# wg-perception/PartsBasedDetector

Measured on AMD Instinct MI355X. Metric: detect() frames/sec, 640x480, 26-part person model, higher is better.
Workload: dtype f32

## Files before the change

### partsbaseddetector_amd/csrc/fold_pick.hpp

```cpp
#pragma once
#include <math.h>

#ifdef __HIPCC__
#define FP_HD __host__ __device__ __forceinline__
#else
#define FP_HD static inline
#endif

template <typename T> struct FoldPick { T v; int i; };

template <typename T, int N = 0>
FP_HD FoldPick<T> fold_pick(const T* sd, const float* bias_col, int K) {
  const int n = N > 0 ? N : K;
  const T w0 = sd[0] + bias_col[0];
  T v = w0 > (T)-INFINITY ? w0 : (T)-INFINITY;
  int bi = 0;
#ifdef __HIPCC__
#pragma unroll
#endif
  for (int k = 1; k < n; ++k) {
    const T wv = sd[k] + bias_col[k];
    const bool take = wv > v;
    bi = take ? k : bi;
    v = take ? wv : v;
  }
  return FoldPick<T>{K == 1 ? w0 : v, bi};
}
```

### partsbaseddetector_amd/csrc/k_dp.hip

```cpp
#include <algorithm>
#include <type_traits>
#include "pbd_internal.hpp"
#include "dt_core.hpp"
#include "fold_pick.hpp"

#define GP(U) const __attribute__((address_space(1))) U*
#define GPW(U) __attribute__((address_space(1))) U*

#ifdef PBD_PROBES
__device__ unsigned long long pbd_dt_dbg[8];
__device__ unsigned long long pbd_dt_cnt[8];
#define DT_COUNT_REDO() do { atomicAdd(&pbd_dt_dbg[7], 1ull); atomicAdd(&pbd_dt_cnt[7], 1ull); } while (0)
#define DT_COUNT(i, c) do { if (c) atomicAdd(&pbd_dt_cnt[i], 1ull); } while (0)
#define DT_COUNT_ROUNDS(n) do { if (threadIdx.x == 0) { atomicAdd(&pbd_dt_cnt[1], (unsigned long long)(n)); \
    atomicMax(&pbd_dt_cnt[2], (unsigned long long)(n)); } } while (0)
#define DT_PROBE_ONLY(...) __VA_ARGS__
#define DT_TRACE_L 40
#define DT_TRACE_B 4096
__device__ unsigned long long pbd_dt_trace[DT_TRACE_L][DT_TRACE_B][8];
__device__ unsigned pbd_dt_trace_hw[DT_TRACE_L][DT_TRACE_B];
__device__ int pbd_dt_trace_launch = DT_TRACE_L;
static int g_dt_trace_seq = 0;
#define DT_STAMP(i) do { if (threadIdx.x == 0) { const unsigned long long now_ = wall_clock64(); if (blockIdx.x == 0) pbd_dt_dbg[i] = now_; \
    if (i && pbd_dt_trace_launch < 40 && blockIdx.x < 4096) pbd_dt_trace[pbd_dt_trace_launch][blockIdx.x][i] = now_; } } while (0)
#define DT_TRACE(k) do { if (threadIdx.x == 0 && pbd_dt_trace_launch < DT_TRACE_L && blockIdx.x < DT_TRACE_B) { \
    pbd_dt_trace[pbd_dt_trace_launch][blockIdx.x][k ? 7 : 0] = wall_clock64(); \
    if (k == 0) { unsigned hw; asm volatile("s_getreg_b32 %0, hwreg(HW_REG_HW_ID)" : "=s"(hw)); unsigned xcc; asm volatile("s_getreg_b32 %0, hwreg(HW_REG_XCC_ID)" : "=s"(xcc)); pbd_dt_trace_hw[pbd_dt_trace_launch][blockIdx.x] = (hw & 0xffffff) | (xcc << 24); } } } while (0)
int dt_debug_trace(unsigned long long* t, unsigned* hw, int* nlaunch) {
  hipMemcpyFromSymbol(t, HIP_SYMBOL(pbd_dt_trace), sizeof(unsigned long long) * DT_TRACE_L * DT_TRACE_B * 8);
  hipMemcpyFromSymbol(hw, HIP_SYMBOL(pbd_dt_trace_hw), sizeof(unsigned) * DT_TRACE_L * DT_TRACE_B);
  *nlaunch = g_dt_trace_seq;
  g_dt_trace_seq = 0;
  return 0;
}
void dt_debug_read(unsigned long long* out) {
  hipMemcpyFromSymbol(out, HIP_SYMBOL(pbd_dt_dbg), sizeof(unsigned long long) * 8);
  const unsigned long long z = 0;
  hipMemcpyToSymbol(HIP_SYMBOL(pbd_dt_dbg), &z, sizeof(z), 7 * sizeof(unsigned long long));
}
void dt_debug_counters(unsigned long long* out) {
  hipMemcpyFromSymbol(out, HIP_SYMBOL(pbd_dt_cnt), sizeof(unsigned long long) * 8);
  const unsigned long long z[8] = {};
  hipMemcpyToSymbol(HIP_SYMBOL(pbd_dt_cnt), z, sizeof(z));
}
#else
#define DT_STAMP(i) do { } while (0)
#define DT_COUNT_REDO() do { } while (0)
#define DT_COUNT(i, c) do { } while (0)
#define DT_COUNT_ROUNDS(n) do { } while (0)
#define DT_PROBE_ONLY(...)
#define DT_TRACE(k) do { } while (0)
void dt_debug_read(unsigned long long* out) { for (int i = 0; i < 8; ++i) out[i] = 0; }
void dt_debug_counters(unsigned long long* out) { for (int i = 0; i < 8; ++i) out[i] = 0; }
#endif

static_assert(offsetof(FoldChild, ok) == 8 * PBD_FOLD_MAXMIX && PBD_FOLD_MAXMIX == 8, "fold_child_qw: sdt[8] then ok");
__device__ __forceinline__ unsigned long long fold_child_qw(const FoldChild* C) {
  return ((GP(unsigned long long))C)[min((int)(threadIdx.x & 63u), 8)];
}
__device__ __forceinline__ GP(char) fold_qw_lane(unsigned long long v, int l) {
  const unsigned lo = (unsigned)__builtin_amdgcn_readlane((int)(unsigned)v, l), hi = (unsigned)__builtin_amdgcn_readlane((int)(unsigned)(v >> 32), l);
  return (GP(char))(((unsigned long long)hi << 32) | lo);
}
template <typename T, int M, int U>
__device__ __forceinline__ void fold_children(const FoldJob* __restrict__ J, const unsigned (&off)[U], T (&acc)[U][M], unsigned long long cv,
                                              int nch) {
  unsigned ob[U];
#pragma unroll
  for (int u = 0; u < U; ++u) ob[u] = off[u] * (unsigned)sizeof(T);
  int c = 0;
  do {
    const FoldChild& C = J->ch[c];
    T sd[U][M];
    unsigned obc[U];
#pragma unroll
    for (int u = 0; u < U; ++u) {
      obc[u] = ob[u];
#if defined(__HIP_DEVICE_COMPILE__)
      asm volatile("" : "+v"(obc[u]));
#endif
    }
#pragma unroll
    for (int k = 0; k < M; ++k) {
      GP(char) pl = fold_qw_lane(cv, k);
#pragma unroll
      for (int u = 0; u < U; ++u) sd[u][k] = *(GP(T))(pl + obc[u]);
    }
    cv = fold_child_qw(&J->ch[min(c + 1, nch - 1)]);
    float bias[M][M];
#pragma unroll
    for (int k = 0; k < M; ++k)
#pragma unroll
      for (int m = 0; m < M; ++m) bias[m][k] = C.bias[k][m];
    const int K = C.K;
#pragma unroll
    for (int u = 0; u < U; ++u)
#pragma unroll
      for (int m = 0; m < M; ++m)
        acc[u][m] = acc[u][m] + fold_pick<T, M>(sd[u], bias[m], K).v;
  } while (++c < nch);
}

template <typename T, typename IT, int FM>
__device__ __forceinline__ void dt_block(char* smem, const DtTask& t, const DtGroup& g, const DtMap* __restrict__ maps,
                                         const FoldJob* __restrict__ folds, const float* __restrict__ biasw,
                                         unsigned long long rawq, unsigned long long c0qw) {

  constexpr bool FOLD = FM > 0;
  const int lane = threadIdx.x, NT = blockDim.x;
  const int len = g.len, S = g.stride, lpb = g.lpb;
  typedef DtPair<T> P2;
  constexpr bool EX = sizeof(T) == 8;
  const bool fz = !EX && (g.fused & DT_G_FUSED) != 0;
  const T** lptr = (const T**)smem;
  int* FLAG = (int*)(smem + lpb * 8);
  int* FIX = FLAG + lpb;
  int* FIX2 = (int*)smem;
  int* SEG = FIX + lpb;
  int* ANY = SEG + DT_SEGS - 6;
  int* NFLAG = SEG + DT_SEGS - 4;
  static_assert(DT_SEGS - 6 > 64, "ANY / NFLAG must lie beyond the P + 1 <= 65 segment starts");
  T* ZLO = (T*)(SEG + DT_SEGS);
  IT* FT = (IT*)(ZLO + NT);
  IT* BELOW = FT + NT;
  IT* DMIN = BELOW + NT;
  IT* BSAVE = DMIN + NT;
  double* RDX = (double*)(smem + dt_hdr_bytes(NT, sizeof(T), sizeof(IT), lpb));
  const int nl = t.nl;
  const int nrows = FOLD ? nl / g.nmaps : 0;
  P2* YZ = (P2*)(RDX + ((S + 1) & ~1));
  IT* B = (IT*)(YZ + lpb * S);
  auto map_line = [&](int i, int& mi, int& li) {
    const int x = t.l0 + i;
    const int q = g.nlines > 1 ? (int)__umulhi((unsigned)x, g.magic_nlines) : x;
    mi = t.m0 + q; li = x - __mul24(q, g.nlines);
  };
  const bool contig = !FOLD && t.src0 != nullptr;
  if (lane < nl) {
    if (!FOLD && !contig) {
      int mi, li;
      map_line(lane, mi, li);
      const DtMap& mp0 = maps[g.map0 + mi];
      lptr[lane] = (const T*)mp0.src + (size_t)li * len;
    }
    FLAG[lane] = 0;
  }
  if (lane < lpb) FIX[lane] = 0x7fffffff;
  const int nsub = g.nsub;
  const int P = g.P;
  if (lane <= P) SEG[lane] = P > 1 ? (int)__umulhi((unsigned)__mul24(lane, len), g.magic_P) : lane * len;
  if (lane == 0) { SEG[DT_SEGS - 2] = 0; SEG[DT_SEGS - 1] = len; ANY[0] = 0; *NFLAG = 0; }
  const int p = lpb > 1 ? (int)__umulhi((unsigned)lane, g.magic_lpb) : lane, line = lane - __mul24(p, lpb);
  const bool mine = line < nl && p < nsub;
  int mi = 0, li = 0;
  if (mine) {
    if (FOLD) {
      const unsigned mrows = nrows > 1 ? (0xFFFFFFFFu / (unsigned)nrows + 1u) : 0u;
      mi = nrows > 1 ? (int)__umulhi((unsigned)line, mrows) : line;
      li = t.g0 + (line - __mul24(mi, nrows));
    } else {
      map_line(line, mi, li);
    }
  }
  DtMap mp;
  P2* YZl = YZ + line * S;
  IT* Bl = B + line * S;
  mp = maps[g.map0 + mi];
  if (!FOLD && !contig) __syncthreads();
  DT_STAMP(1);
  if constexpr (FOLD) {
    constexpr int M = FM > 0 ? FM : 1;
    constexpr int U = sizeof(T) == 8 ? 1 : 3;
    const FoldJob* J = folds + g.fold;
    const int L = g.nmaps;
    GP(char) srcp[M];
#pragma unroll
    for (int m = 0; m < M; ++m) srcp[m] = fold_qw_lane(rawq, m);
    const int nch0 = __builtin_amdgcn_readlane((int)(unsigned)c0qw, 9);
    const int n = nrows * len;
    const unsigned cell0 = (unsigned)t.g0 * (unsigned)len;
    const unsigned magic = len > 1 ? (0xFFFFFFFFu / (unsigned)len + 1u) : 0u;
    for (int e0 = 0; e0 < n; e0 += NT * U) {
// ... 61 lines not shown
  __syncthreads();
  DT_STAMP(2);

  if (mine && p < P) {
    const bool sus = fz ? dt_seg_scan<EX, !EX, T, IT>(YZl, Bl, RDX, mp.r2a, SEG[p], SEG[p + 1], mp.a, mp.b)
                        : dt_seg_scan<EX, false, T, IT>(YZl, Bl, RDX, mp.r2a, SEG[p], SEG[p + 1], mp.a, mp.b);
    if (sus) { FLAG[line] = 1; *NFLAG = 1; }
  }
  __syncthreads();
  DT_STAMP(3);
  DT_PROBE_ONLY(const bool scan_flagged = mine && p == 0 && FLAG[line]; DT_COUNT(5, scan_flagged);)
  T zs_mine = (T)0;
  const bool stitched = mine && p >= 1 && p < P && !FLAG[line];
  if (stitched) {
    int f, dmin, bs;
    T zs;
    const bool bad = fz ? dt_stitch1<EX, !EX, T, IT>(YZl, Bl, RDX, mp.r2a, SEG[p], SEG[p + 1], mp.a, mp.b, f, dmin, zs, bs)
                        : dt_stitch1<EX, false, T, IT>(YZl, Bl, RDX, mp.r2a, SEG[p], SEG[p + 1], mp.a, mp.b, f, dmin, zs, bs);
    FT[lane] = (IT)f; DMIN[lane] = (IT)dmin; zs_mine = zs; BSAVE[lane] = (IT)bs;
    if (bad) { FLAG[line] = 1; *NFLAG = 1; }
  }
  if (mine && p == 0) FT[lane] = (IT)0;
  __syncthreads();
  {
    const bool cand = mine && p >= 2 && p < P;
    const bool live = mine && p < P && !FLAG[line];
    const int fspec_prev = cand ? (int)FT[lane - lpb] : 0;
    if (cand && live && dt_stitch_stale((int)DMIN[lane], fspec_prev, fspec_prev)) { atomicMin(&FIX[line], p); ANY[0] = 1; }
    if (live) {
      const int f = (int)FT[lane];
      BELOW[lane] = Bl[f];
      ZLO[lane] = YZl[f].y;
    }
    __syncthreads();
    DT_STAMP(6);
    if (ANY[0]) {
      DT_COUNT(0, lane == 0);
      if (stitched) ZLO[lane] = zs_mine;
      __syncthreads();
      for (int round = 0;; ++round) {
        int* FIXr = (round & 1) ? FIX2 : FIX;
        int* FIXn = (round & 1) ? FIX : FIX2;
        if (mine && p == 0 && FIXr[line] != 0x7fffffff) {
          const int ps = FIXr[line], ls = __mul24(ps, lpb) + line;
          int f, bs = (int)BSAVE[ls];
          T zs = ZLO[ls];
          const bool bad = fz ? dt_stitch_redo<EX, !EX, T, IT>(YZl, Bl, RDX, mp.r2a, SEG[ps], SEG[ps + 1], mp.a, mp.b, (int)FT[ls], f, zs, bs)
                              : dt_stitch_redo<EX, false, T, IT>(YZl, Bl, RDX, mp.r2a, SEG[ps], SEG[ps + 1], mp.a, mp.b, (int)FT[ls], f, zs, bs);
          FT[ls] = (IT)f; BSAVE[ls] = (IT)bs;
          DMIN[ls] = (IT)SEG[ps];
          DT_COUNT(3, true);
          if (bad) { FLAG[line] = 1; *NFLAG = 1; }
        }
        if (lane < lpb) FIXn[lane] = 0x7fffffff;
        if (lane == 0) ANY[(round + 1) & 1] = 0;
        __syncthreads();
        if (cand && !FLAG[line] && dt_stitch_stale((int)DMIN[lane], fspec_prev, (int)FT[lane - lpb])) { atomicMin(&FIXn[line], p); ANY[(round + 1) & 1] = 1; }
        DT_COUNT(4, cand && !FLAG[line] && (int)DMIN[lane] > fspec_prev && (int)DMIN[lane] <= (int)FT[lane - lpb]);
        __syncthreads();
        if (!ANY[(round + 1) & 1]) { DT_COUNT_ROUNDS(round + 1); break; }
      }
      if (mine && p < P && !FLAG[line]) {
        const int f = (int)FT[lane];
        BELOW[lane] = Bl[f];
        ZLO[lane] = YZl[f].y;
      }
      __syncthreads();
    }
  }
  if (*NFLAG) {
    if (mine && p == 0 && FLAG[line]) {
      DT_COUNT_REDO();
      DT_COUNT(6, !scan_flagged);
      dt_seg_scan<true, false, T, IT>(YZl, Bl, RDX, mp.r2a, 0, len, mp.a, mp.b);
      BELOW[line] = Bl[0];
      ZLO[line] = YZl[0].y;
    }
    __syncthreads();
  }
  DT_STAMP(4);

  if (mine) {
    const double a = mp.a, b = mp.b;
    int16_t* pp = mp.ptr + li;
    const int chunk = g.chunk;
    const int q0 = p * chunk, q1 = min(len, q0 + chunk);
    if (q0 < q1) {
      int os = mp.os + q1 - 1;
      const bool whole = FLAG[line] != 0;
      int e = dt_cover<T, IT>(YZl, Bl, whole ? SEG + DT_SEGS - 2 : SEG, whole ? 1 : P, BELOW + line, ZLO + line, lpb, os);
      P2 eyz = YZl[e];
      int nx = (int)Bl[e];
      P2 nyz = YZl[nx];
      int nnx = (int)Bl[nx];
      const int nlines = g.nlines;
      GPW(T) dp = (GPW(T))mp.dst + li + (size_t)(q1 - 1) * nlines;
      GPW(int16_t) ppq = (GPW(int16_t))pp + (size_t)(q1 - 1) * nlines;
      const int os_end = mp.os + q0;
      ++os;
      auto outputs = [&](auto fused) {
        constexpr bool FZ = decltype(fused)::value;
        do {
          --os;
          const T fos = (T)os;
          while (!(eyz.y < fos)) { e = nx; eyz = nyz; nx = nnx; nyz = YZl[nx]; nnx = (int)Bl[nx]; }
          const double d = (double)(os - e);
          const double ad2 = a * (d * d);
          *dp = (T)((FZ ? fma(b, d, ad2) : (ad2 + b * d)) + (double)eyz.x);
          *ppq = (int16_t)e;
          dp -= nlines; ppq -= nlines;
        } while (os > os_end);
      };
      if constexpr (!EX) { if (fz) outputs(std::true_type{}); else outputs(std::false_type{}); }
      else outputs(std::false_type{});
    }
  }
  DT_STAMP(5);
}

template <typename T, int FM>
__global__ __launch_bounds__(256, 3) void k_dt_pass(const DtTask* __restrict__ tasks, const DtMap* __restrict__ maps,
                                                    const FoldJob* __restrict__ folds, const float* __restrict__ biasw,
                                                    const unsigned long long* __restrict__ foldx) {
  extern __shared__ __attribute__((aligned(16))) char smem[];
#if PBD_DT_PRIO > 0
  __builtin_amdgcn_s_setprio(PBD_DT_PRIO);
#endif
  DT_STAMP(0);
  DT_TRACE(0);
#if PBD_DT_TASK_PREFETCH > 0 && defined(__HIP_DEVICE_COMPILE__)
  unsigned pf_off = 0;
  asm("" : "+v"(pf_off));
  const unsigned pf_val = *(const unsigned*)((const char*)(tasks + min(blockIdx.x + (unsigned)PBD_DT_TASK_PREFETCH, gridDim.x - 1u)) + pf_off);
#endif
  unsigned long long rawq = 0, c0qw = 0;
  if constexpr (FM > 0) {
    GP(unsigned long long) fx = (GP(unsigned long long))foldx + (size_t)blockIdx.x * PBD_FOLDX_QW;
    const int l = (int)(threadIdx.x & 63u);
    rawq = fx[min(l, 7)];
    c0qw = fx[8 + min(l, 9)];
  }
  const DtTask t = tasks[blockIdx.x];
  const DtGroup& g = t.g;
  if (g.stride <= 256) dt_block<T, unsigned char, FM>(smem, t, g, maps, folds, biasw, rawq, c0qw);
  else dt_block<T, unsigned short, FM>(smem, t, g, maps, folds, biasw, rawq, c0qw);
  DT_TRACE(1);
#if PBD_DT_TASK_PREFETCH > 0 && defined(__HIP_DEVICE_COMPILE__)
  asm volatile("" :: "v"(pf_val));
#endif
}

template <typename T, int FM>
static void launch_dt_pass_t(const DtTask* tasks, int ntasks, const DtMap* maps, const FoldJob* folds, const unsigned long long* foldx, const float* biasw,
                             size_t lds, int nt, hipStream_t s) {
  static LdsOptIn optin;
  optin.ensure((const void*)k_dt_pass<T, FM>, lds);
#ifdef PBD_PROBES
  static const bool tracing = getenv("PBD_DT_TRACE") != nullptr;
  if (tracing) { static int seqs[4096]; const int seq = g_dt_trace_seq++; seqs[seq & 4095] = seq; hipMemcpyToSymbolAsync(HIP_SYMBOL(pbd_dt_trace_launch), &seqs[seq & 4095], sizeof(int), 0, hipMemcpyHostToDevice, s); }
#endif
  hipLaunchKernelGGL((k_dt_pass<T, FM>), dim3(ntasks), dim3(nt), lds, s, tasks, maps, folds, biasw, foldx);
}
template <typename T>
static void launch_dt_pass_m(const DtTask* tasks, int ntasks, const DtMap* maps, const FoldJob* folds, const unsigned long long* foldx, const float* biasw,
                             size_t lds, int nt, int fm, hipStream_t s) {
  if (!folds) launch_dt_pass_t<T, 0>(tasks, ntasks, maps, folds, foldx, biasw, lds, nt, s);
  else if (fm <= 1) launch_dt_pass_t<T, 1>(tasks, ntasks, maps, folds, foldx, biasw, lds, nt, s);
  else if (fm <= 4) launch_dt_pass_t<T, 4>(tasks, ntasks, maps, folds, foldx, biasw, lds, nt, s);
  else if (fm <= 6) launch_dt_pass_t<T, 6>(tasks, ntasks, maps, folds, foldx, biasw, lds, nt, s);
  else launch_dt_pass_t<T, PBD_FOLD_MAXMIX>(tasks, ntasks, maps, folds, foldx, biasw, lds, nt, s);
}
void launch_dt_pass(const DtTask* tasks, int ntasks, const DtMap* maps, const FoldJob* folds, const unsigned long long* foldx, const float* biasw, size_t lds,
                    int ts, int nt, int fm, hipStream_t s) {
  if (ntasks <= 0) return;
  if (ts == 8) launch_dt_pass_m<double>(tasks, ntasks, maps, folds, foldx, biasw, lds, nt, fm, s);
  else launch_dt_pass_m<float>(tasks, ntasks, maps, folds, foldx, biasw, lds, nt, fm, s);
}

template <typename T>
__global__ __launch_bounds__(256) void k_reduce(const ReduceJob* __restrict__ jobs, const ReduceBlock* __restrict__ blocks,
                                                const float* __restrict__ biasw, int correct_ptr) {
  __shared__ ReduceJob J;
  const ReduceBlock rb = blocks[blockIdx.x];
  {
    const int* src = (const int*)(jobs + rb.job);
    int* dst = (int*)&J;
    for (int i = threadIdx.x; i < (int)(sizeof(ReduceJob) / 4); i += 256) dst[i] = src[i];
  }
  __syncthreads();
  const unsigned cell = rb.cell0 + threadIdx.x;
  const int H = J.H, W = J.W, L = J.L;
  const unsigned HW = (unsigned)H * W;
  if (cell >= HW) return;
  constexpr int ML = 8;
  if (L <= ML) {
    T acc[ML];
#pragma unroll
// ... 112 lines not shown
    }
    return;
  }
  const int K = J.K;
  if (J.fold >= 0) {
    constexpr int M = FM;
    T acc[1][M];
    const unsigned long long c0qw = fold_child_qw(&folds[J.fold].ch[0]);
    const unsigned cellc = live ? cell : HWr - 1u;
    const unsigned offs[1] = {cellc};
#pragma unroll
    for (int m = 0; m < M; ++m) acc[0][m] = ((GP(T))J.score[m])[cellc];
    fold_children<T, M, 1>(folds + J.fold, offs, acc, c0qw, folds[J.fold].nch);
    if (!live) return;
    if (K == 1) {
      v = acc[0][0] + bias;
    } else {
      v = -INFINITY;
#pragma unroll
      for (int m = 0; m < M; ++m) {
        if (m < K) {
          const T wv = acc[0][m] + bias;
          if (wv > v) { bi = m; v = wv; }
        }
      }
    }
  } else if (K == 1) {
    v = ((const T*)J.score[0])[cell] + bias;
  } else {
    v = -INFINITY;
    for (int m = 0; m < K; ++m) {
      const T wv = ((const T*)J.score[m])[cell] + bias;
      if (wv > v) { bi = m; v = wv; }
    }
  }
  ((T*)J.rootv)[cell] = v;
  J.rooti[cell] = bi;
  if ((double)v > thresh) {
    const int idx = atomicAdd(count, 1);
    if (idx < capacity) {
      CandRec r;
      r.level = J.level; r.comp = J.comp; r.y = cell / J.W; r.x = cell - r.y * J.W;
      rec[idx] = r;
    }
  }
}

template <typename T>
static void launch_root_t(const RootJob* jobs, const ReduceBlock* blocks, int nblocks, double thresh, int* count, CandRec* rec,
                          int capacity, const FoldJob* folds, const float* biasw, int rescan, int fm, const uint8_t* nms_mask,
                          const char* rootv_base, hipStream_t s) {
  const dim3 g(nblocks), b(256);
  if (fm <= 1) hipLaunchKernelGGL((k_root<T, 1>), g, b, 0, s, jobs, blocks, thresh, count, rec, capacity, folds, biasw, rescan, nms_mask, rootv_base);
  else if (fm <= 4) hipLaunchKernelGGL((k_root<T, 4>), g, b, 0, s, jobs, blocks, thresh, count, rec, capacity, folds, biasw, rescan, nms_mask, rootv_base);
  else if (fm <= 6) hipLaunchKernelGGL((k_root<T, 6>), g, b, 0, s, jobs, blocks, thresh, count, rec, capacity, folds, biasw, rescan, nms_mask, rootv_base);
  else hipLaunchKernelGGL((k_root<T, PBD_FOLD_MAXMIX>), g, b, 0, s, jobs, blocks, thresh, count, rec, capacity, folds, biasw, rescan, nms_mask, rootv_base);
}
void launch_root(const RootJob* jobs, const ReduceBlock* blocks, int nblocks, double thresh, int* count, CandRec* rec,
                 int capacity, int ts, const FoldJob* folds, const float* biasw, int rescan, int fm, const uint8_t* nms_mask,
                 const char* rootv_base, hipStream_t s) {
  if (nblocks <= 0) return;
  if (ts == 8) launch_root_t<double>(jobs, blocks, nblocks, thresh, count, rec, capacity, folds, biasw, rescan, fm, nms_mask, rootv_base, s);
  else launch_root_t<float>(jobs, blocks, nblocks, thresh, count, rec, capacity, folds, biasw, rescan, fm, nms_mask, rootv_base, s);
}

#define BT_MAXP 256
struct BtChild { GP(char) sdt[PBD_FOLD_MAXMIX]; GP(FoldChild) C; int K; };
__device__ __forceinline__ BtChild bt_child(const char* folds, const unsigned long long* __restrict__ pick, size_t i) {
  BtChild c;
  c.C = (GP(FoldChild))(folds + pick[i]);
#pragma unroll
  for (int k = 0; k < PBD_FOLD_MAXMIX; ++k) c.sdt[k] = (GP(char))c.C->sdt[k];
  c.K = c.C->K;
  return c;
}
template <typename T>
__global__ __launch_bounds__(64) void k_backtrack(const int* __restrict__ count, const CandRec* __restrict__ rec,
                                                  int capacity, const BackLevel* __restrict__ back, int ncomp,
                                                  const int* __restrict__ parent, const int* __restrict__ plane0,
                                                  const int* __restrict__ nparts, int max_parts, const int* __restrict__ mix_rows,
                                                  char* __restrict__ out, size_t out_stride,
                                                  const int* __restrict__ flat, const int* __restrict__ depth, int max_depth,
                                                  int nflat, const unsigned long long* __restrict__ scr_base,
                                                  const int16_t* __restrict__ ixs, const int16_t* __restrict__ iys,
                                                  int correct_ptr, const int16_t* __restrict__ extx,
                                                  const int16_t* __restrict__ exty, const unsigned long long* __restrict__ ext_base,
                                                  int* __restrict__ count_out, int org,
                                                  const char* __restrict__ folds, const unsigned long long* __restrict__ pick) {
  __shared__ int lx[BT_MAXP], ly[BT_MAXP], lm[BT_MAXP];
  const int lane = threadIdx.x;
  const int n = min(*count, capacity);
  if (count_out && blockIdx.x == 0 && lane == 0) *count_out = *count;
  for (int idx = blockIdx.x; idx < n; idx += gridDim.x) {
  __syncthreads();
  const CandRec r = rec[idx];
  const BackLevel B = back[r.level * ncomp + r.comp];
  const size_t HW = (size_t)B.H * B.W;
  char* o = out + (size_t)idx * out_stride;
  pbd_candidate_head* head = (pbd_candidate_head*)o;
  int32_t* boxes = (int32_t*)(o + sizeof(pbd_candidate_head));
  int32_t* locs = boxes + (size_t)max_parts * 4;
  const int np = nparts[r.comp];
  if (lane == 0) {
    head->score = (float)((const T*)B.rootv)[(size_t)r.y * B.W + r.x];
    head->component = r.comp;
    head->level = r.level;
    head->nparts = np;
    lx[0] = r.x; ly[0] = r.y; lm[0] = B.rooti[(size_t)r.y * B.W + r.x];
  }
  BtChild ch0{};
  if (pick && lane >= 1 && lane < np) ch0 = bt_child(folds, pick, (size_t)r.level * nflat + flat[r.comp * max_parts + lane]);
  __syncthreads();
  for (int d = 1; d <= max_depth; ++d) {
    for (int p = lane; p < np; p += 64) {
      if (depth[r.comp * max_parts + p] != d) continue;
      const int par = parent[r.comp * max_parts + p];
      const int px = lx[par], py = ly[par], pm = lm[par];
      const size_t off = (size_t)py * B.W + px;
      int mm;
      if (pick) {
        const BtChild ch = p == lane ? ch0 : bt_child(folds, pick, (size_t)r.level * nflat + flat[r.comp * max_parts + p]);
        T sd[PBD_FOLD_MAXMIX];
        float bc[PBD_FOLD_MAXMIX];
#pragma unroll
        for (int k = 0; k < PBD_FOLD_MAXMIX; ++k) {
          sd[k] = ((GP(T))ch.sdt[k])[off];
          bc[k] = ch.C->bias[k][pm];
        }
        mm = fold_pick<T, PBD_FOLD_MAXMIX>(sd, bc, ch.K).i;
      } else {
        mm = B.pk[(size_t)(plane0[r.comp * max_parts + p] + pm) * HW + off];
      }
      int x, y;
      if (extx) {
        const size_t eo = (size_t)ext_base[r.level * ncomp + r.comp] + (size_t)(plane0[r.comp * max_parts + p] + pm) * HW + off;
        x = extx[eo]; y = exty[eo];
      } else {
        const size_t so = (size_t)scr_base[(size_t)r.level * nflat + flat[r.comp * max_parts + p]] + (size_t)mm * HW;
        if (!correct_ptr) { x = ixs[so + (size_t)px * B.H + py]; y = iys[so + (size_t)py * B.W + x]; }
        else { y = iys[so + off]; x = ixs[so + (size_t)px * B.H + y]; }
      }
      lx[p] = x; ly[p] = y; lm[p] = mm;
    }
    __syncthreads();
  }
  const T scale = B.scale;
  for (int p = lane; p < max_parts; p += 64) {
    if (p < np) {
      const int sz = t_round((T)mix_rows[flat[r.comp * max_parts + p] * PBD_MAX_MIX + (lm[p] & (PBD_MAX_MIX - 1))] * scale);
      const int x = lx[p], y = ly[p];
      locs[p * 3] = x; locs[p * 3 + 1] = y; locs[p * 3 + 2] = lm[p];
      const int x1 = t_round((T)(x - org) * scale), y1 = t_round((T)(y - org) * scale);
      const int x2 = x1 + sz - 1, y2 = y1 + sz - 1;
      boxes[p * 4] = min(x1, x2); boxes[p * 4 + 1] = min(y1, y2);
      boxes[p * 4 + 2] = max(x1, x2) - min(x1, x2); boxes[p * 4 + 3] = max(y1, y2) - min(y1, y2);
    } else {
      for (int k = 0; k < 4; ++k) boxes[p * 4 + k] = 0;
      for (int k = 0; k < 3; ++k) locs[p * 3 + k] = 0;
    }
  }
  }
}

void launch_backtrack(const int* count, const CandRec* rec, int capacity, const BackLevel* back, int ncomp,
                      const int* parent, const int* plane0, const int* nparts, int max_parts, const int* mix_rows, char* out,
                      size_t out_stride, int ts, const int* flat, const int* depth, int max_depth, int nflat,
                      const unsigned long long* scr_base, const int16_t* ix, const int16_t* iy, int correct_ptr,
                      const int16_t* extx, const int16_t* exty, const unsigned long long* ext_base, int* count_out, int pad,
                      const FoldJob* folds, const unsigned long long* pick, hipStream_t s) {
  const int nblk = std::min(capacity, 2048);
  if (ts == 8) hipLaunchKernelGGL(k_backtrack<double>, dim3(nblk), dim3(64), 0, s, count, rec, capacity, back, ncomp, parent, plane0, nparts, max_parts, mix_rows, out, out_stride, flat, depth, max_depth, nflat, scr_base, ix, iy, correct_ptr, extx, exty, ext_base, count_out, 1 + pad, (const char*)folds, pick);
  else hipLaunchKernelGGL(k_backtrack<float>, dim3(nblk), dim3(64), 0, s, count, rec, capacity, back, ncomp, parent, plane0, nparts, max_parts, mix_rows, out, out_stride, flat, depth, max_depth, nflat, scr_base, ix, iy, correct_ptr, extx, exty, ext_base, count_out, 1 + pad, (const char*)folds, pick);
}

template <typename T>
__device__ __forceinline__ void nms_block(const T* __restrict__ src, int M, int N, int sz, uint8_t* __restrict__ dst, int b) {
  const int nbx = (N + sz) / (sz + 1), nby = (M + sz) / (sz + 1);
  if (b >= nbx * nby) return;
  const int m = (b / nbx) * (sz + 1), n = (b % nbx) * (sz + 1);
  const int i1 = min(m + sz + 1, M), j1 = min(n + sz + 1, N);
  double vcmax = -1.7976931348623157e308;
  int ci = m, cj = n;
  for (int i = m; i < i1; ++i)
    for (int j = n; j < j1; ++j) {
      const double v = src[(size_t)i * N + j];
      if (v > vcmax) { vcmax = v; ci = i; cj = j; }
    }
  const int in0 = max(ci - sz, 0), in1 = min(ci + sz + 1, M);
  const int jn0 = max(cj - sz, 0), jn1 = min(cj + sz + 1, N);
  const int is0 = m - in0, is1 = min(m - in0 + sz + 1, in1 - in0);
  const int js0 = n - jn0, js1 = min(n - jn0 + sz + 1, jn1 - jn0);
  double vnmax = -1.7976931348623157e308;
  bool any = false;
  for (int i = in0; i < in1; ++i)
    for (int j = jn0; j < jn1; ++j) {
      const int li = i - in0, lj = j - jn0;
      if (li >= is0 && li < is1 && lj >= js0 && lj < js1) continue;
      any = true;
      const double v = src[(size_t)i * N + j];
      if (v > vnmax) vnmax = v;
    }
  if (!any) vnmax = 0;
  if (vcmax > vnmax) dst[(size_t)ci * N + cj] = 255;
}
__global__ __launch_bounds__(64) void k_nms_map(const float* __restrict__ src, int M, int N, int sz,
                                                uint8_t* __restrict__ dst) {
  nms_block<float>(src, M, N, sz, dst, blockIdx.x * 64 + threadIdx.x);
}
template <typename T>
__global__ __launch_bounds__(64) void k_nms_roots(const RootJob* __restrict__ jobs, const char* __restrict__ rootv_base, int sz,
                                                  uint8_t* __restrict__ mask) {
  const RootJob& J = jobs[blockIdx.y];
  nms_block<T>((const T*)J.rootv, J.H, J.W, sz, mask + (size_t)((const char*)J.rootv - rootv_base) / sizeof(T), blockIdx.x * 64 + threadIdx.x);
}
void launch_nms_roots(const RootJob* jobs, int njobs, unsigned maxcells, const char* rootv_base, int ts, int sz, uint8_t* mask, hipStream_t s) {
  if (njobs <= 0 || maxcells == 0) return;
  const dim3 grid((maxcells + 63) / 64, njobs);
  if (ts == 8) hipLaunchKernelGGL(k_nms_roots<double>, grid, dim3(64), 0, s, jobs, rootv_base, sz, mask);
  else hipLaunchKernelGGL(k_nms_roots<float>, grid, dim3(64), 0, s, jobs, rootv_base, sz, mask);
}

void launch_nms_map(const float* src, int rows, int cols, int sz, uint8_t* dst, hipStream_t s) {
  const int nb = ((cols + sz) / (sz + 1)) * ((rows + sz) / (sz + 1));
  hipMemsetAsync(dst, 0, (size_t)rows * cols, s);
  hipLaunchKernelGGL(k_nms_map, dim3((nb + 63) / 64), dim3(64), 0, s, src, rows, cols, sz, dst);
}
```

### partsbaseddetector_amd/csrc/pbd_api.cpp

```cpp
#include <algorithm>
#include <cmath>
#include <cstddef>
#include <cstdio>
#include <cstring>
#include <new>
#include "pbd_internal.hpp"
#include "pbd_split.hpp"

static int upload_bank(pbd_handle* h, const float* filt, int nf, int kh, int kw, SizeGroup& g, size_t* bytes) {
  const pbd_model_desc& m = h->md;
  g.kh = kh; g.kw = kw; g.nf = nf;
  g.nfpad = ((nf + 159) / 160) * 160;
  const size_t wt_n = (size_t)kh * kw * m.flen * g.nfpad;
  std::vector<float> wT(3 * wt_n + m.flen, 0.f);
  wT[wt_n + m.flen - 1] = 1.f;
  if (m.flen == PBD_FLEN)
    for (int n = 0; n < nf; ++n)
      for (int tap = 0; tap < kh * kw; ++tap)
        for (int c = 0; c < m.flen; ++c)
        {
          const float w = filt[((size_t)n * kh * kw + tap) * m.flen + c];
          wT[wt_n + m.flen + ((((size_t)tap * 2 + c / 16) * 4 + (c % 16) / 4) * g.nfpad + n) * 4 + c % 4] = w;
          wT[2 * wt_n + m.flen + ((((size_t)tap * 2 + c / 16) * 4 + c % 4) * g.nfpad + n) * 4 + (c % 16) / 4] = w;
        }
// ... 157 lines not shown
  h->d_cf_mask = nullptr; h->cf_mask_bytes = 0;
  h->d_ik_blocks = nullptr; h->d_ik_cells = nullptr; h->n_ik_blocks = 0;
  h->d_lat_jobs = nullptr; h->d_lat_blocks = nullptr; h->d_lat_flags = nullptr; h->d_lat_partial = nullptr; h->n_lat_blocks = 0;
  h->fw = h->fh = h->fcn = 0; h->fdepth = 0; h->fesz = 1; h->ldepth = 0; h->lesz = 1;
  h->d_matjobs = nullptr; h->d_matruns = nullptr; h->d_mattaps = nullptr;
  reset_stages(h);
  h->feat_split_ok = false;
}

static bool all_active_set(const pbd_handle* h, const std::vector<char>& v, int per_level) {
  if (v.size() != (size_t)h->nvl * per_level) return false;
  for (int l = 0; l < h->nvl; ++l) {
    if (!h->lv[l].active || h->lv[l].cw == 0 || h->lv[l].ch == 0) continue;
    for (int k = 0; k < per_level; ++k) if (!v[(size_t)l * per_level + k]) return false;
  }
  return true;
}

static PlanKnobs read_plan_knobs() {
  PlanKnobs k;
  if (const char* e = PBD_PROBE_ENV("PBD_DT_NT")) k.dt_nt = std::max(64, std::min(256, atoi(e) & ~63));
  if (const char* e = PBD_PROBE_ENV("PBD_DT_SEG")) k.dt_seg = atoi(e);
  if (const char* e = PBD_PROBE_ENV("PBD_DT_BUDGET_KB")) k.dt_budget_kb = atoi(e);
  if (const char* e = PBD_PROBE_ENV("PBD_DT_BUDGET_B")) k.dt_budget_b = atoi(e);
  if (const char* e = PBD_PROBE_ENV("PBD_DT_XCD_CHUNK")) k.xcd_chunk = atoi(e);
  return k;
}

int plan_frame(pbd_handle* h, int w, int hgt, int cn, int batch, int depth) {
  if (h->fw == w && h->fh == hgt && h->fcn == cn && h->batch == batch && h->fdepth == depth) return PBD_OK;
  if (cn != 1 && cn != 3) return fail(h, PBD_ERR_UNSUPPORTED, "image: 1 or 3 channels");
  const int esz = depth_esz(depth);
  if (!esz) return fail(h, PBD_ERR_UNSUPPORTED, "Unsupported image type (src/HOGFeatures.cpp:136-146: CV_8U, CV_16U, CV_32F, CV_64F)");
  if (esz > 1 && batch != 1) return fail(h, PBD_ERR_UNSUPPORTED, "batches of frames: 8-bit images");
  if (batch < 1 || batch > 64) return fail(h, PBD_ERR_ARG, "batch: 1..64 frames");
  hipStreamSynchronize(h->stream);
  free_frame(h);
  FrameSpec fs;
  fs.w = w; fs.h = hgt; fs.cn = cn; fs.batch = batch; fs.depth = depth; fs.level_set = h->level_set;
  FrameLayout lay;
  int rc = plan_layout(*h, fs, lay, &h->err);
  if (rc) return rc;
  std::vector<char*> regions(lay.regions.size(), nullptr);
  for (size_t i = 0; i < regions.size(); ++i)
    if ((rc = dev_alloc(h, &regions[i], lay.regions[i]))) return rc;
  const FrameBases b = frame_bases(lay, regions.data());
  int ncu = 256;
  { hipDeviceProp_t pr; if (hipGetDeviceProperties(&pr, h->opt.device) == hipSuccess && pr.multiProcessorCount > 0) ncu = pr.multiProcessorCount; }
  h->ncu = ncu;
  FrameTables t;
  if ((rc = plan_tables(*h, fs, lay, b, ncu, h->dt_geom, h->knobs, t, &h->err))) return rc;
  if ((rc = dev_upload(h, &h->d_pyrjobs, t.pyrjobs)) || (rc = dev_upload(h, &h->d_levels, t.levels)) ||
      (h->pyr_kind == PBD_PYRAMID_MATLAB && ((rc = dev_upload(h, &h->d_matjobs, t.matjobs)) || (rc = dev_upload(h, &h->d_matruns, t.matruns)) ||
                                             (rc = dev_upload(h, &h->d_mattaps, t.mattaps)))) ||
      (h->pad > 0 && ((rc = dev_upload(h, &h->d_hog_levels, t.hog_levels)) || (rc = dev_upload(h, &h->d_padjobs, t.padjobs)) ||
                      (rc = dev_upload(h, &h->d_padblocks, t.padblk)))) ||
      (rc = dev_upload(h, &h->d_hog_tiles, t.hog_tiles)) || (rc = dev_upload(h, &h->d_conv_tiles, t.conv_tiles)) ||
      (h->mixed && (rc = dev_upload(h, &h->d_conv_tiles_mix, t.conv_tiles_mix))) ||
      (rc = dev_upload(h, &h->d_dtmaps, t.maps)) || (rc = dev_upload(h, &h->d_dttasks, t.tasks)) ||
      (rc = dev_upload(h, &h->d_foldjobs, t.folds)) || (rc = dev_upload(h, &h->d_foldx, t.foldx)) ||
      (rc = dev_upload(h, &h->d_redjobs, t.red)) || (rc = dev_upload(h, &h->d_redblocks, t.redblk)) ||
      (rc = dev_upload(h, &h->d_rootjobs, t.rootjobs)) || (rc = dev_upload(h, &h->d_rootblocks, t.rootblk)) ||
      (rc = dev_upload(h, &h->d_back, t.back)) || (rc = dev_upload(h, &h->d_scr_base, t.scr_base)) ||
      (rc = dev_upload(h, &h->d_pick, t.pick)))
    return rc;
  {
    const size_t nflat = h->parts.size();
    std::vector<ReduceBlock> blocks;
    std::vector<unsigned> cells(t.pick.size(), 0);
    for (size_t i = 0; i < t.pick.size(); ++i) {
      if (t.pick[i] == PBD_NO_PICK) continue;
      const Level& L = lay.lv[i / nflat];
      cells[i] = (unsigned)L.cw * (unsigned)L.ch;
      for (unsigned c0 = 0; c0 < cells[i]; c0 += 256) blocks.push_back(ReduceBlock{(int)i, c0});
    }
    if ((rc = dev_upload(h, &h->d_ik_cells, cells)) || (rc = dev_upload(h, &h->d_ik_blocks, blocks))) return rc;
    h->n_ik_blocks = (int)blocks.size();
  }
  h->lv = lay.lv; h->nlevels = lay.nlevels; h->batch = batch; h->nvl = lay.nvl;
  h->first_copy = kFirstCopy * batch;
  h->cells = lay.cells; h->pyr_bytes = lay.pyr_bytes; h->compact = lay.compact; h->dt_cap_elems = lay.dt_cap_elems;
  h->d_img = (uint8_t*)b.p[FB_IMG]; h->d_pyr = (uint8_t*)b.p[FB_PYR]; h->d_feat = b.p[FB_FEAT]; h->d_resp = b.p[FB_RESP];
  h->d_pk = (uint8_t*)b.p[FB_PK]; h->d_rootv = b.p[FB_ROOTV]; h->d_rooti = (int*)b.p[FB_ROOTI]; h->d_nms_mask = (uint8_t*)b.p[FB_NMS_MASK];
  h->d_dt_tmpT = b.p[FB_DT_TMPT]; h->d_dt_sdt = b.p[FB_DT_SDT]; h->d_dt_ixT = (int16_t*)b.p[FB_DT_IXT]; h->d_dt_iy = (int16_t*)b.p[FB_DT_IY];
  h->d_acc = b.p[FB_ACC]; h->d_feat_split = (uint16_t*)b.p[FB_FEAT_SPLIT];
  h->pyr_launches = std::move(t.pyr_launches);
  if (h->pad == 0) { h->d_hog_levels = h->d_levels; h->d_padjobs = nullptr; h->d_padblocks = nullptr; }
  h->n_padblocks = (int)t.padblk.size();
  h->hog_tc = t.hog_tc; h->n_hog_tiles = (int)t.hog_tiles.size(); h->n_conv_tiles = (int)t.conv_tiles.size();
  h->dt_nt = t.dt_nt; h->dt_lds = t.dt_lds;
  h->rl = std::move(t.rl);
  h->n_rootjobs = (int)t.rootjobs.size(); h->n_rootblocks = (int)t.rootblk.size();
  h->root_cells = t.root_cells; h->root_maxcells = t.root_maxcells;
  h->scr_base = std::move(t.scr_base);
  h->fw = w; h->fh = hgt; h->fcn = cn; h->fdepth = depth; h->fesz = esz;
  h->lesz = lay.esz; h->ldepth = h->pyr_kind == PBD_PYRAMID_MATLAB ? PBD_DEPTH_64F : depth;
  return PBD_OK;
}
static int run_image_pyramid(pbd_handle* h, const uint8_t* d_src, int stride) {
  for (size_t i = 0; i < h->pyr_launches.size(); ++i) {
    const PyrLaunch& P = h->pyr_launches[i];
    if (h->pyr_kind == PBD_PYRAMID_MATLAB) {
      if (i == 0) launch_resize_area(h->d_matjobs + P.job0, P.njobs, P.maxpix, h->d_matruns, h->d_mattaps, h->fcn, stride, false, d_src, h->d_pyr, h->stream);
      else launch_reduce_f64(h->d_matjobs + P.job0, P.njobs, P.maxpix, h->fcn, h->d_pyr, h->stream);
    } else
    if (h->fdepth != PBD_DEPTH_8U) {
      if (i == 0) launch_resize_any(h->d_pyrjobs + P.job0, P.njobs, P.maxpix, h->fcn, h->fdepth, stride, d_src, h->d_pyr, h->stream);
      else launch_pyrdown_any(h->d_pyrjobs + P.job0, P.njobs, P.maxpix, h->fcn, h->fdepth, h->d_pyr, h->stream);
    } else
    if (i == 0) launch_resize(h->d_pyrjobs + P.job0, P.njobs, P.maxpix, h->fcn, stride, d_src, h->d_pyr, h->stream);
    else launch_pyrdown(h->d_pyrjobs + P.job0, P.njobs, P.maxw, P.maxh, h->fcn, h->d_pyr, h->stream);
  }
  LAUNCHCHK(h, "image pyramid");
  mark_pyramid(h);
  return PBD_OK;
}

static int run_hog(pbd_handle* h) {
  uint16_t* split = h->split_parts ? h->d_feat_split : nullptr;
  launch_hog(h->d_hog_tiles, h->n_hog_tiles, h->d_hog_levels, h->d_pyr, h->d_feat, h->ts, h->fcn, h->md.sbin, h->hog_tc, h->d_hog_lut, split, h->split_parts, h->ldepth, h->stream);
  if (h->pad > 0) launch_featpad(h->d_padjobs, h->d_padblocks, h->n_padblocks, h->d_feat, h->ts, split, h->split_parts, h->stream);
  LAUNCHCHK(h, "HOG");
  mark_features(h, split != nullptr);
  return PBD_OK;
}

static void ensure_feat_split(pbd_handle* h) {
  if (!h->split_parts || h->feat_split_ok) return;
  if (h->split_parts == 2) launch_feat_split16((const float*)h->d_feat, h->d_feat_split, h->cells, h->stream);
  else launch_feat_split((const float*)h->d_feat, h->d_feat_split, h->cells, h->stream);
  h->feat_split_ok = true;
}

static void launch_bank(pbd_handle* h, const ConvTile* tiles, int nf, int nfpad, int kh, int kw, const void* wT, const uint16_t* wS,
                        const float* oscale, int nf_stride) {
  const size_t wt_n = (size_t)kh * kw * h->md.flen * nfpad, cell = h->md.flen;
  if (h->conv_mode == PBD_CONV_SPLIT_F16)
    launch_conv_split16(tiles, h->n_conv_tiles, h->d_levels, h->d_feat_split, wS, (float*)h->d_resp, nf, kh, kw, oscale, h->stream, nf_stride);
  else if (h->conv_mode == PBD_CONV_SPLIT)
    launch_conv_split(tiles, h->n_conv_tiles, h->d_levels, h->d_feat_split, wS, (float*)h->d_resp, nf, kh, kw, h->stream, nf_stride);
  else if (h->conv_mode == PBD_CONV_MFMA && h->ts == 8)
    launch_conv_mfma_f64(tiles, h->n_conv_tiles, h->d_levels, (const double*)h->d_feat, (const double*)wT + wt_n + cell, (double*)h->d_resp, nf, nfpad, kh, kw, h->stream, nf_stride);
  else if (h->conv_mode == PBD_CONV_MFMA)
    launch_conv_mfma16_f32(tiles, h->n_conv_tiles, h->d_levels, (const float*)h->d_feat, (const float*)wT + 2 * wt_n + cell, (float*)h->d_resp, nf, nfpad, kh, kw, h->stream, nf_stride);
  else
    launch_conv_exact(tiles, h->n_conv_tiles, h->d_levels, h->d_feat, wT, h->d_resp, h->ts, nf, nfpad, kh, kw, h->stream, nf_stride);
}

#if defined(PBD_TUNE) || defined(PBD_PROBES)
bool launch_conv_variant(const pbd_handle* h);
#else
static bool launch_conv_variant(const pbd_handle*) { return false; }
#endif

static int run_pdf(pbd_handle* h) {
  const pbd_model_desc& m = h->md;
  ensure_feat_split(h);
  const bool variant_ran = launch_conv_variant(h);
  if (h->mixed) {
    for (size_t gi = 0; gi < h->groups.size(); ++gi) {
      const SizeGroup& g = h->groups[gi];
      launch_bank(h, h->d_conv_tiles_mix + gi * h->n_conv_tiles, g.nf, g.nfpad, g.kh, g.kw, g.d_wT, g.d_wS, g.d_oscale, m.nfilters);
    }
  } else if (!variant_ran) {
    launch_bank(h, h->d_conv_tiles, m.nfilters, h->nfpad, m.kh, m.kw, h->d_wT, h->d_wS, h->d_split_oscale, 0);
  }
  LAUNCHCHK(h, "filter bank");
// ... 91 lines not shown
          const int fid = h->parts[p0 + p].filterid[k];
          LatJob J{};
          J.plane = h->d_resp + (L.cell_off * h->md.nfilters + (size_t)fid * HW) * h->ts;
          J.H = L.ch; J.W = L.cw; J.level = l; J.comp = c; J.part = p; J.mix = k;
          J.rows = h->mixed ? h->fkh[fid] : h->md.kh;
          J.flag = (l * nc + c) * mp + p;
          J.scale = L.scale;
          for (size_t c0 = 0; c0 < HW; c0 += 256) blocks.push_back(ReduceBlock{(int)jobs.size(), (unsigned)c0});
          jobs.push_back(J);
        }
    }
  }
  int rc;
  if ((rc = dev_upload(h, &h->d_lat_jobs, jobs)) || (rc = dev_upload(h, &h->d_lat_blocks, blocks)) ||
      (rc = dev_alloc(h, &h->d_lat_flags, (size_t)h->nvl * nc * mp)) || (rc = dev_alloc(h, &h->d_lat_partial, (size_t)std::max(h->n_rootblocks, 1))))
    return rc;
  h->n_lat_blocks = (int)blocks.size();
  return PBD_OK;
}

int pbd_i_latent_begin(pbd_handle* h, const LatentSource& s, int nframes) {
  int rc = latent_tables(h);
  if (rc) return rc;
  const int mp = h->max_parts;
  const size_t cap = (size_t)PBD_MAX_BATCH * mp * 5;
  if (!h->d_lat_truth && ((rc = model_alloc(h, &h->d_lat_truth, cap)) || (rc = model_alloc(h, &h->h_lat_truth, cap, true, false)))) return rc;
  const size_t nt = (size_t)nframes * mp * 4, nm = (size_t)nframes * mp;
  memcpy(h->h_lat_truth, s.truth, nt * sizeof(int));
  if (s.mix) memcpy(h->h_lat_truth + nt, s.mix, nm * sizeof(int));
  HIPCHK(h, hipMemcpyAsync(h->d_lat_truth, h->h_lat_truth, (nt + (s.mix ? nm : 0)) * sizeof(int), hipMemcpyHostToDevice, h->stream));
  h->lat_has_mix = s.mix != nullptr;
  h->lat_component = s.component; h->lat_overlap = s.overlap;
  return PBD_OK;
}

static int run_latent_mask(pbd_handle* h, int nframes) {
  const int nc = h->md.ncomponents, mp = h->max_parts;
  hipMemsetAsync(h->d_lat_flags, 0, (size_t)h->nvl * nc * mp * sizeof(int), h->stream);
  LatentMaskArgs a{};
  a.jobs = h->d_lat_jobs; a.blocks = h->d_lat_blocks;
  a.truth = h->d_lat_truth; a.mix = h->lat_has_mix ? h->d_lat_truth + (size_t)nframes * mp * 4 : nullptr;
  a.flags = h->d_lat_flags;
  a.nlevels = h->nlevels; a.mp = mp; a.component = h->lat_component; a.org = 1 + h->pad;
  a.overlap = h->lat_overlap;
  launch_latent_mask(a, h->n_lat_blocks, h->ts, h->stream);
  LAUNCHCHK(h, "latent mask");
  mark_latent_mask(h, h->lat_component);
  return PBD_OK;
}
static int run_latent_best(pbd_handle* h) {
  LatentBestArgs a{};
  a.jobs = h->d_rootjobs; a.blocks = h->d_rootblocks; a.nblocks = h->n_rootblocks;
  a.flags = h->d_lat_flags; a.nparts = h->d_nparts;
  a.ncomp = h->md.ncomponents; a.mp = h->max_parts; a.nlevels = h->nlevels; a.nframes = h->batch;
  a.partial = h->d_lat_partial;
  a.count = h->d_cand_count; a.rec = h->d_cand_rec;
  launch_latent_best(a, h->ts, h->stream);
  LAUNCHCHK(h, "latent best");
  return PBD_OK;
}

static int run_argmin_enqueue(pbd_handle* h, bool filter = false) {
  if (h->root_dirty) {
    hipMemsetAsync(h->d_cand_count, 0, sizeof(int), h->stream);
    if (h->nms_sz > 0) nms_and_rescan(h);
    else
    launch_root(h->d_rootjobs, h->d_rootblocks, h->n_rootblocks, (double)h->md.thresh, h->d_cand_count, h->d_cand_rec,
                h->opt.max_candidates, h->ts, h->d_foldjobs, h->d_biasw, 1, h->fold_mix, nullptr, nullptr, h->stream);
    h->root_dirty = false;
  }
  const int cm = filter ? pbd_i_cand_mode(h) : PBD_CAND_RAW;
  h->out_filtered = cm != PBD_CAND_RAW;
  const bool zf = filter && h->zf_frame && h->zf_on;
  const bool post = zf || h->out_filtered;
  const bool zero_copy = PBD_ARGMIN_ZERO_COPY && !h->d_gsend;
  char* out = h->h_cand_out;
  int* count_out = h->h_cand_count;
  if (post || !zero_copy) {
    out = post && (zf || h->d_gsend) ? h->d_cand_raw : h->d_cand_out;
    count_out = nullptr;
  }
  launch_backtrack(h->d_cand_count, h->d_cand_rec, h->opt.max_candidates, h->d_back, h->md.ncomponents, h->d_parent,
                   h->d_plane0, h->d_nparts, h->max_parts, h->d_mix_rows, out, h->cand_stride, h->ts, h->d_flat,
                   h->d_depth, h->max_depth, (int)h->parts.size(), h->d_scr_base, h->d_dt_ixT, h->d_dt_iy,
                   h->opt.dt_correct_ptr, h->ext_ptr ? h->d_extx : nullptr, h->d_exty, h->d_ext_base, count_out, h->pad,
                   h->d_foldjobs, h->ik_lazy && !h->ext_ptr ? h->d_pick : nullptr, h->stream);
  if (post) return pbd_i_post_enqueue(h, cm, zf, out);
  LAUNCHCHK(h, "argmin");
  if (zero_copy) { h->pending = true; h->out_on_host = true; return PBD_OK; }
  h->out_on_host = false;
  if (h->d_gsend || h->first_copy < kFirstCopy * h->batch) h->first_copy = kFirstCopy * h->batch;
  const int first = std::min(h->first_copy, h->opt.max_candidates);
  if (h->d_gsend) {
    HIPCHK(h, hipMemcpyAsync(h->d_gsend, h->d_cand_count, sizeof(int), hipMemcpyDeviceToDevice, h->stream));
    HIPCHK(h, hipMemcpyAsync(h->d_gsend + 16, h->d_cand_out, h->cand_stride * first, hipMemcpyDeviceToDevice, h->stream));
  } else {
    HIPCHK(h, hipMemcpyAsync(h->h_cand_count, h->d_cand_count, sizeof(int), hipMemcpyDeviceToHost, h->stream));
    HIPCHK(h, hipMemcpyAsync(h->h_cand_out, h->d_cand_out, h->cand_stride * first, hipMemcpyDeviceToHost, h->stream));
  }
  h->pending = true;
  return PBD_OK;
}

static int enqueue_stages(pbd_handle* h, const uint8_t* d_src, int stride) {
  int rc;
  const bool prof = h->profiling;
  if (prof) hipEventRecord(h->ev[0], h->stream);
  if ((rc = run_image_pyramid(h, d_src, stride))) return rc;
  if (prof) hipEventRecord(h->ev[1], h->stream);
  if ((rc = run_hog(h))) return rc;
  if (prof) hipEventRecord(h->ev[2], h->stream);
  if ((rc = run_pdf(h))) return rc;
  if (h->lat_frame && (rc = run_latent_mask(h, h->batch))) return rc;
  if (prof) hipEventRecord(h->ev[3], h->stream);
  if ((rc = run_dp_min(h))) return rc;
  if (h->lat_frame && (rc = run_latent_best(h))) return rc;
  if (prof) hipEventRecord(h->ev[4], h->stream);
  if ((rc = run_argmin_enqueue(h, true))) return rc;
  if (h->lat_frame) h->root_dirty = true;
  if (prof) hipEventRecord(h->ev[5], h->stream);
  if (h->ps_frame && (rc = pbd_i_run_part_scores(h))) return rc;
  if (h->b3_frame && (rc = pbd_i_run_box3d(h))) return rc;
  return PBD_OK;
}

int enqueue_all(pbd_handle* h, const uint8_t* d_src, int stride) {
  const bool graphable = h->opt.graph && !h->profiling;
  int rc = pbd_i_post_buffers(h);
  if (rc) return rc;
  if (h->zf_frame || h->lat_frame) return enqueue_stages(h, d_src, stride);
  if (!graphable || h->frames_on_plan == 0) {
    h->frames_on_plan++;
    return enqueue_stages(h, d_src, stride);
  }
  const size_t row = (size_t)h->fw * h->fcn * h->fesz;
  if (d_src != h->d_img && (rc = copy_rows(h, h->d_img, d_src, (size_t)stride, row, (size_t)h->fh * h->batch, hipMemcpyDeviceToDevice))) return rc;
  if (!h->gexec) {
    hipGraph_t graph = nullptr;
    HIPCHK(h, hipStreamBeginCapture(h->stream, hipStreamCaptureModeThreadLocal));
    rc = enqueue_stages(h, h->d_img, (int)row);
    hipError_t e = hipStreamEndCapture(h->stream, &graph);
    if (rc) { if (graph) hipGraphDestroy(graph); return rc; }
    if (e != hipSuccess) return fail(h, PBD_ERR_HIP, std::string("hipStreamEndCapture: ") + hipGetErrorString(e));
    e = hipGraphInstantiate(&h->gexec, graph, nullptr, nullptr, 0);
    hipGraphDestroy(graph);
    if (e != hipSuccess) { h->gexec = nullptr; return fail(h, PBD_ERR_HIP, std::string("hipGraphInstantiate: ") + hipGetErrorString(e)); }
  }
  HIPCHK(h, hipGraphLaunch(h->gexec, h->stream));
  h->frames_on_plan++;
  mark_pyramid(h);
  mark_features(h, h->split_parts != 0);
  mark_responses(h);
  mark_min(h, false);
  h->pending = true;
  return PBD_OK;
}

void read_stage_times(pbd_handle* h) {
  if (!h->profiling) return;
  for (int i = 0; i < 5; ++i) hipEventElapsedTime(&h->stage_ms[i], h->ev[i], h->ev[i + 1]);
  hipEventElapsedTime(&h->stage_ms[5], h->ev[0], h->ev[5]);
}

static_assert(sizeof(pbd_camera) == 48, "pbd_camera layout");
static_assert(sizeof(pbd_box3d) == 80 && offsetof(pbd_box3d, zmin) == 20 && offsetof(pbd_box3d, x3d) == 32, "pbd_box3d layout");
static_assert(sizeof(pbd_part_score) == 24 && offsetof(pbd_part_score, bias) == 16, "pbd_part_score layout");
static_assert(sizeof(pbd_cluster3d) == 40 && offsetof(pbd_cluster3d, first) == 12 && offsetof(pbd_cluster3d, cx) == 16,
// ... 249 lines not shown
  HIPCHK(h, hipMemcpy(out, h->d_feat + L.cell_off * PBD_FLEN * ts, (size_t)L.cw * L.ch * PBD_FLEN * ts, hipMemcpyDeviceToHost));
  return PBD_OK;
}
int pbd_get_frame_level_features(pbd_handle* h, int frame, int level, float* out) { return get_frame_level_features_(h, frame, level, out, 4); }
int pbd_get_frame_level_features_f64(pbd_handle* h, int frame, int level, double* out) { return get_frame_level_features_(h, frame, level, out, 8); }
int pbd_get_level_features(pbd_handle* h, int level, float* out) { return get_level_features_(h, level, out, 4); }
int pbd_get_level_features_f64(pbd_handle* h, int level, double* out) { return get_level_features_(h, level, out, 8); }
int pbd_set_level_features(pbd_handle* h, int level, const float* in) { return set_level_features_(h, level, in, 4); }
int pbd_set_level_features_f64(pbd_handle* h, int level, const double* in) { return set_level_features_(h, level, in, 8); }
int pbd_pdf(pbd_handle* h) {
  if (!h) return PBD_ERR_ARG;
  if (!h->have_feat) return fail(h, PBD_ERR_STATE, h->compact ? "pdf(): features are not resident (compact memory plan: min() reuses their memory — run pyramid() or hand in every level again)" : "pdf() before pyramid()");
  ON_DEVICE(h);
  int rc = run_pdf(h);
  if (rc) return rc;
  HIPCHK(h, hipStreamSynchronize(h->stream));
  return PBD_OK;
}
static int get_level_response_(pbd_handle* h, int level, int filter, void* out, int ts) {
  CHECK_LEVEL(h, level);
  CHECK_SCALAR(h, ts);
  if (!h->have_resp) return fail(h, PBD_ERR_STATE, "responses not computed");
  if (filter < 0 || filter >= h->md.nfilters) return fail(h, PBD_ERR_ARG, "filter out of range");
  if (!h->fperm.empty()) filter = h->fperm[filter];
  const Level& L = h->lv[level];
  if (!L.active) return fail(h, PBD_ERR_STATE, "level is not processed by this handle (pbd_set_levels / level_begin..level_end)");
  const size_t HW = (size_t)L.cw * L.ch;
  ON_DEVICE(h);
  HIPCHK(h, hipStreamSynchronize(h->stream));
  HIPCHK(h, hipMemcpy(out, h->d_resp + (L.cell_off * h->md.nfilters + filter * HW) * ts, HW * ts, hipMemcpyDeviceToHost));
  return PBD_OK;
}
static int set_level_response_(pbd_handle* h, int level, int filter, const void* in, int ts) {
  CHECK_LEVEL(h, level);
  CHECK_SCALAR(h, ts);
  if (filter < 0 || filter >= h->md.nfilters) return fail(h, PBD_ERR_ARG, "filter out of range");
  if (!h->fperm.empty()) filter = h->fperm[filter];
  const Level& L = h->lv[level];
  const size_t HW = (size_t)L.cw * L.ch;
  if (!in) return fail(h, PBD_ERR_ARG, "null response map");
  if ((ts == 4 ? pbd_first_nonfinite((const float*)in, HW) : pbd_first_nonfinite((const double*)in, HW)) != HW)
    return fail(h, PBD_ERR_ARG, "non-finite response: the distance transform takes finite scores only");
  ON_DEVICE(h);
  if (h->compact) { int rc = ensure_ik(h); if (rc) return rc; }
  HIPCHK(h, hipStreamSynchronize(h->stream));
  HIPCHK(h, hipMemcpy(h->d_resp + (L.cell_off * h->md.nfilters + filter * HW) * ts, in, HW * ts, hipMemcpyHostToDevice));
  if (h->compact) {
    if (h->resp_ok.size() != (size_t)h->nvl * h->md.nfilters) compact_mark_resp(h, false);
    h->resp_ok[(size_t)level * h->md.nfilters + filter] = 1;
    h->have_resp = all_active_set(h, h->resp_ok, h->md.nfilters);
    h->lat_masked = false;
  } else {
    mark_responses(h);
  }
  return PBD_OK;
}
int pbd_get_level_response(pbd_handle* h, int level, int filter, float* out) { return get_level_response_(h, level, filter, out, 4); }
int pbd_get_level_response_f64(pbd_handle* h, int level, int filter, double* out) { return get_level_response_(h, level, filter, out, 8); }
int pbd_set_level_response(pbd_handle* h, int level, int filter, const float* in) { return set_level_response_(h, level, filter, in, 4); }
int pbd_set_level_response_f64(pbd_handle* h, int level, int filter, const double* in) { return set_level_response_(h, level, filter, in, 8); }
int pbd_dp_min(pbd_handle* h) {
  if (!h) return PBD_ERR_ARG;
  if (!h->have_resp) return fail(h, PBD_ERR_STATE, h->compact ? "min(): responses are not resident (compact memory plan: min() transforms them in place — run pdf() or hand in every plane again)" : "min() before pdf()");
  ON_DEVICE(h);
  int rc = run_dp_min(h);
  if (!rc) rc = ensure_ik(h);
  if (rc) return rc;
  HIPCHK(h, hipStreamSynchronize(h->stream));
  return PBD_OK;
}
static int get_dp_pointers_(pbd_handle* h, int level, int component, int part, int parent_mix, int32_t* ix, int32_t* iy, int32_t* ik) {
  if (!h->have_dp) return fail(h, PBD_ERR_STATE, "min() not run");
  if (component < 0 || component >= h->md.ncomponents) return fail(h, PBD_ERR_ARG, "component out of range");
  const int p0 = h->part_offset[component], cnp = h->part_offset[component + 1] - p0;
  if (part < 1 || part >= cnp) return fail(h, PBD_ERR_ARG, "part out of range (1..nparts-1)");
  const PartInfo& P = h->parts[p0 + part];
  const int L_ = h->parts[p0 + P.parent].K;
  if (parent_mix < 0 || parent_mix >= L_) return fail(h, PBD_ERR_ARG, "parent mixture out of range");
  const Level& L = h->lv[level];
  const size_t HW = (size_t)L.cw * L.ch;
  const size_t po = L.cell_off * h->nplanes + (size_t)(P.plane0 + parent_mix) * HW;
  if (!L.active) return fail(h, PBD_ERR_STATE, "level is not processed by this handle");
  std::vector<uint8_t> c(HW);
  std::vector<int16_t> X((size_t)P.K * HW), Y((size_t)P.K * HW);
  const size_t so = (size_t)h->scr_base[(size_t)level * h->parts.size() + (p0 + part)];
  ON_DEVICE(h);
  { int rc = ensure_ik(h); if (rc) return rc; }
  HIPCHK(h, hipStreamSynchronize(h->stream));
  HIPCHK(h, hipMemcpy(c.data(), h->d_pk + po, HW, hipMemcpyDeviceToHost));
  HIPCHK(h, hipMemcpy(X.data(), h->d_dt_ixT + so, X.size() * 2, hipMemcpyDeviceToHost));
  HIPCHK(h, hipMemcpy(Y.data(), h->d_dt_iy + so, Y.size() * 2, hipMemcpyDeviceToHost));
  const int W = L.cw, H = L.ch;
  for (size_t i = 0; i < HW; ++i) {
    const size_t mo = (size_t)c[i] * HW;
    const int m_ = (int)(i / W), n_ = (int)(i - (size_t)m_ * W);
    int x, y;
    if (!h->opt.dt_correct_ptr) { x = X[mo + (size_t)n_ * H + m_]; y = Y[mo + (size_t)m_ * W + x]; }
    else { y = Y[mo + i]; x = X[mo + (size_t)n_ * H + y]; }
    if (ix) ix[i] = x;
    if (iy) iy[i] = y;
    if (ik) ik[i] = c[i];
  }
  return PBD_OK;
}
int pbd_get_dp_pointers(pbd_handle* h, int level, int component, int part, int parent_mix, int32_t* ix, int32_t* iy, int32_t* ik) {
  CHECK_LEVEL(h, level);
  return get_dp_pointers_(h, level, component, part, parent_mix, ix, iy, ik);
}
int pbd_get_frame_dp_pointers(pbd_handle* h, int frame, int level, int component, int part, int parent_mix, int32_t* ix, int32_t* iy, int32_t* ik) {
  CHECK_FRAME_LEVEL(h, frame, level);
  return get_dp_pointers_(h, frame * h->nlevels + level, component, part, parent_mix, ix, iy, ik);
}
static int get_root_(pbd_handle* h, int level, int component, void* rootv, int32_t* rooti, int ts) {
  CHECK_LEVEL(h, level);
  CHECK_SCALAR(h, ts);
  if (!h->have_dp) return fail(h, PBD_ERR_STATE, "min() not run");
  if (component < 0 || component >= h->md.ncomponents) return fail(h, PBD_ERR_ARG, "component out of range");
  const Level& L = h->lv[level];
  if (!L.active) return fail(h, PBD_ERR_STATE, "level is not processed by this handle (pbd_set_levels / level_begin..level_end)");
  const size_t HW = (size_t)L.cw * L.ch;
  ON_DEVICE(h);
  HIPCHK(h, hipStreamSynchronize(h->stream));
  if (rootv) HIPCHK(h, hipMemcpy(rootv, h->d_rootv + (L.cell_off * h->md.ncomponents + component * HW) * ts, HW * ts, hipMemcpyDeviceToHost));
  if (rooti) HIPCHK(h, hipMemcpy(rooti, h->d_rooti + L.cell_off * h->md.ncomponents + component * HW, HW * 4, hipMemcpyDeviceToHost));
  return PBD_OK;
}
int pbd_get_root(pbd_handle* h, int level, int component, float* rootv, int32_t* rooti) { return get_root_(h, level, component, rootv, rooti, 4); }
int pbd_get_root_f64(pbd_handle* h, int level, int component, double* rootv, int32_t* rooti) { return get_root_(h, level, component, rootv, rooti, 8); }
static int set_root_(pbd_handle* h, int level, int component, const void* rootv, const int32_t* rooti, int ts) {
  CHECK_LEVEL(h, level);
  CHECK_SCALAR(h, ts);
  if (component < 0 || component >= h->md.ncomponents) return fail(h, PBD_ERR_ARG, "component out of range");
  const Level& L = h->lv[level];
  if (!L.active) return fail(h, PBD_ERR_STATE, "level is not processed by this handle (pbd_set_levels / level_begin..level_end)");
  const size_t HW = (size_t)L.cw * L.ch;
  if (rooti) {
    const int K0 = h->parts[h->part_offset[component]].K;
    for (size_t i = 0; i < HW; ++i)
      if (rooti[i] < 0 || rooti[i] >= K0) return fail(h, PBD_ERR_ARG, "rooti entry out of range (0..K_root-1)");
  }
  ON_DEVICE(h);
  HIPCHK(h, hipStreamSynchronize(h->stream));
  if (rootv) HIPCHK(h, hipMemcpy(h->d_rootv + (L.cell_off * h->md.ncomponents + component * HW) * ts, rootv, HW * ts, hipMemcpyHostToDevice));
  if (rooti) HIPCHK(h, hipMemcpy(h->d_rooti + L.cell_off * h->md.ncomponents + component * HW, rooti, HW * 4, hipMemcpyHostToDevice));
  h->root_dirty = true;
  if (rootv && rooti) {
    if (h->root_set.size() != (size_t)h->nvl * h->md.ncomponents) h->root_set.assign((size_t)h->nvl * h->md.ncomponents, 0);
    h->root_set[(size_t)level * h->md.ncomponents + component] = 1;
  }
  return PBD_OK;
}
int pbd_set_root(pbd_handle* h, int level, int component, const float* rootv, const int32_t* rooti) { return set_root_(h, level, component, rootv, rooti, 4); }
int pbd_set_root_f64(pbd_handle* h, int level, int component, const double* rootv, const int32_t* rooti) { return set_root_(h, level, component, rootv, rooti, 8); }
int pbd_set_dp_pointers(pbd_handle* h, int level, int component, int part, int parent_mix, const int32_t* ix, const int32_t* iy, const int32_t* ik) {
  CHECK_LEVEL(h, level);
  if (!ix || !iy || !ik) return fail(h, PBD_ERR_ARG, "null table");
  if (component < 0 || component >= h->md.ncomponents) return fail(h, PBD_ERR_ARG, "component out of range");
  const int p0 = h->part_offset[component], cnp = h->part_offset[component + 1] - p0;
  if (part < 1 || part >= cnp) return fail(h, PBD_ERR_ARG, "part out of range (1..nparts-1)");
  const PartInfo& P = h->parts[p0 + part];
  if (parent_mix < 0 || parent_mix >= h->parts[p0 + P.parent].K) return fail(h, PBD_ERR_ARG, "parent mixture out of range");
  const Level& L = h->lv[level];
  if (!L.active) return fail(h, PBD_ERR_STATE, "level is not processed by this handle");
  const size_t HW = (size_t)L.cw * L.ch;
  ON_DEVICE(h);
  { int rc = ensure_ik(h); if (rc) return rc; }
  HIPCHK(h, hipStreamSynchronize(h->stream));
  if (!h->d_extx) {
    const size_t n = h->cells * (size_t)std::max(h->nplanes, 1);
    int rc;
    if ((rc = dev_alloc(h, &h->d_extx, n))) return rc;
    if ((rc = dev_alloc(h, &h->d_exty, n))) return rc;
    HIPCHK(h, hipMemset(h->d_extx, 0, n * sizeof(int16_t)));
    HIPCHK(h, hipMemset(h->d_exty, 0, n * sizeof(int16_t)));
    std::vector<unsigned long long> base((size_t)h->nvl * h->md.ncomponents);
    for (int l = 0; l < h->nvl; ++l)
      for (int c = 0; c < h->md.ncomponents; ++c)
        base[(size_t)l * h->md.ncomponents + c] = h->lv[l].cell_off * h->nplanes + (size_t)h->comp_plane0[c] * h->lv[l].cw * h->lv[l].ch;
    if ((rc = dev_upload(h, &h->d_ext_base, base))) return rc;
  }
  if (!h->ext_ptr && h->have_dp && h->min_ran) {
// ... 53 lines not shown
  return PBD_OK;
}

static int argmin_ready(pbd_handle* h) {
  if (!h->have_dp) return fail(h, PBD_ERR_STATE, "argmin() before min()");
  if (h->batch > 1) return fail(h, PBD_ERR_STATE, "the current plan is a batch of frames: its candidates come from pbd_detect_batch_collect");
  if (h->pending) return fail(h, PBD_ERR_STATE, "previous frame not collected");
  if (!h->min_ran) {
    if (!all_active_set(h, h->ext_set, std::max(h->nplanes, 1)) && h->nplanes > 0)
      return fail(h, PBD_ERR_STATE, "argmin(): no min() on this frame and not every pointer table has been handed in (pbd_set_dp_pointers)");
    if (!all_active_set(h, h->root_set, h->md.ncomponents))
      return fail(h, PBD_ERR_STATE, "argmin(): no min() on this frame and not every root table has been handed in (pbd_set_root)");
  }
  return PBD_OK;
}

int pbd_dp_argmin(pbd_handle* h, pbd_candidate_head* heads, int32_t* boxes, int32_t* locs, int capacity, int* count) {
  if (!h) return PBD_ERR_ARG;
  int ready = argmin_ready(h);
  if (ready) return ready;
  ON_DEVICE(h);
  h->ps_frame = h->ps_ready = false;
  int rc = run_argmin_enqueue(h);
  if (rc) { h->pending = false; return rc; }
  return collect_frame(h, heads, boxes, locs, capacity, count);
}

int pbd_latent_mask(pbd_handle* h, const int32_t* truth, const int32_t* mix, int component, double overlap, int32_t* admissible) {
  if (!h) return PBD_ERR_ARG;
  if (h->pending) return fail(h, PBD_ERR_STATE, "a frame is in flight: collect it first");
  int rc = pbd_i_latent_check(h, truth, mix, 1, component, overlap);
  if (rc) return rc;
  if (h->fw == 0) return fail(h, PBD_ERR_STATE, "no frame geometry");
  if (h->batch > 1) return fail(h, PBD_ERR_STATE, "the current plan is a batch of frames (pbd_detect_batch_*): the stage entry points address single-frame plans");
  if (!h->have_resp) return fail(h, PBD_ERR_STATE, h->compact ? "latent mask: responses are not resident (compact memory plan: min() transforms them in place — run pdf() or hand in every plane again)" : "latent mask before pdf()");
  ON_DEVICE(h);
  const LatentSource s{truth, mix, component, overlap};
  if ((rc = pbd_i_latent_begin(h, s, 1)) || (rc = run_latent_mask(h, 1))) return rc;
  HIPCHK(h, hipStreamSynchronize(h->stream));
  if (admissible) {
    const int nc = h->md.ncomponents, mp = h->max_parts;
    std::vector<int> fl((size_t)h->nvl * nc * mp);
    HIPCHK(h, hipMemcpy(fl.data(), h->d_lat_flags, fl.size() * sizeof(int), hipMemcpyDeviceToHost));
    for (int l = 0; l < h->nlevels; ++l)
      for (int c = 0; c < nc; ++c) {
        int ok = 1;
        for (int p = 0; p < h->part_offset[c + 1] - h->part_offset[c]; ++p) ok = ok && fl[((size_t)l * nc + c) * mp + p] != 0;
        admissible[(size_t)l * nc + c] = ok;
      }
  }
  return PBD_OK;
}
int pbd_dp_argbest(pbd_handle* h, pbd_candidate_head* head, int32_t* boxes, int32_t* locs, int* found) {
  if (!h) return PBD_ERR_ARG;
  int rc = argmin_ready(h);
  if (rc) return rc;
  if (h->in_group) return fail(h, PBD_ERR_UNSUPPORTED, "latent detection: not for a pbd_group member");
  if (h->nms_sz > 0) return fail(h, PBD_ERR_UNSUPPORTED, "latent detection: not with the score-map NMS (pbd_options.reserved[0] > 0)");
  ON_DEVICE(h);
  if ((rc = latent_tables(h))) return rc;
  if (!h->lat_masked)
    HIPCHK(h, hipMemsetAsync(h->d_lat_flags, 1, (size_t)h->nvl * h->md.ncomponents * h->max_parts * sizeof(int), h->stream));
  h->ps_frame = h->ps_ready = false;
  if ((rc = run_latent_best(h))) return rc;
  h->root_dirty = false;
  rc = run_argmin_enqueue(h);
  h->root_dirty = true;
  if (rc) { h->pending = false; return rc; }
  return collect_frame(h, head, boxes, locs, 1, found);
}

static int dt2d_(pbd_handle* h, const void* in, int rows, int cols, double ax, double bx, double ay, double by, int osx,
                 int osy, void* out, int32_t* ix, int32_t* iy, int tsz) {
  if (!h || !in || rows <= 0 || cols <= 0 || rows > 32767 || cols > 32767) return PBD_ERR_ARG;
  CHECK_SCALAR(h, tsz);
  if (ax == 0 || ay == 0) return fail(h, PBD_ERR_ARG, "a must be non-zero");
  if (!std::isfinite(ax) || !std::isfinite(bx) || !std::isfinite(ay) || !std::isfinite(by)) return fail(h, PBD_ERR_ARG, "a and b must be finite");
  const size_t HW = (size_t)rows * cols;
  if ((tsz == 4 ? pbd_first_nonfinite((const float*)in, HW) : pbd_first_nonfinite((const double*)in, HW)) != HW)
    return fail(h, PBD_ERR_ARG, "non-finite score: the distance transform takes finite maps only");
  ON_DEVICE(h);
  const size_t ts = (size_t)tsz;
  char *d_in, *d_tmp, *d_sdt;
  int16_t *d_ixT, *d_iy;
  HIPCHK(h, hipMalloc(&d_in, HW * ts)); HIPCHK(h, hipMalloc(&d_tmp, HW * ts)); HIPCHK(h, hipMalloc(&d_sdt, HW * ts));
  HIPCHK(h, hipMalloc(&d_ixT, HW * 2)); HIPCHK(h, hipMalloc(&d_iy, HW * 2));
  HIPCHK(h, hipMemcpyAsync(d_in, in, HW * ts, hipMemcpyHostToDevice, h->stream));
  DtMap maps[2] = {dt_map(d_in, d_tmp, d_ixT, 0.f, 0.f, osx, 1), dt_map(d_tmp, d_sdt, d_iy, 0.f, 0.f, osy, 0)};
  maps[0].a = ax; maps[0].b = bx; maps[0].r2a = 1.0 / (2.0 * ax);
  maps[1].a = ay; maps[1].b = by; maps[1].r2a = 1.0 / (2.0 * ay);
  const int nt = h->knobs.dt_nt ? h->knobs.dt_nt : tsz == 8 ? 64 : PBD_DT_NT_DEFAULT;
  const size_t dt_base = h->knobs.dt_budget_kb >= 0 ? (size_t)h->knobs.dt_budget_kb * 1024 : 40 * 1024;
  const size_t budget = std::max<size_t>(dt_base, dt_lds_bytes(dt_stride_for(std::max(rows, cols)), 4, tsz, nt));
  if (budget > 160 * 1024) return fail(h, PBD_ERR_UNSUPPORTED, "map too large for the LDS-resident distance transform");
  DtGroup groups[2] = {dt_group(0, 1, rows, cols, budget, tsz, nt, h->knobs.dt_seg, true), dt_group(1, 1, cols, rows, budget, tsz, nt, h->knobs.dt_seg, false)};
  std::vector<DtTask> tasks;
  dt_add_tasks(groups[0], tasks);
  const int nx = (int)tasks.size();
  dt_add_tasks(groups[1], tasks);
  dt_mark_fused(tasks, maps, tsz);
  DtMap* d_maps; DtTask* d_tasks;
  HIPCHK(h, hipMalloc(&d_maps, sizeof(maps)));
  HIPCHK(h, hipMalloc(&d_tasks, sizeof(DtTask) * tasks.size()));
  HIPCHK(h, hipMemcpyAsync(d_maps, maps, sizeof(maps), hipMemcpyHostToDevice, h->stream));
  HIPCHK(h, hipMemcpyAsync(d_tasks, tasks.data(), sizeof(DtTask) * tasks.size(), hipMemcpyHostToDevice, h->stream));
  HIPCHK(h, hipStreamSynchronize(h->stream));
  launch_dt_pass(d_tasks, nx, d_maps, nullptr, nullptr, h->d_biasw, budget, tsz, nt, 0, h->stream);
  if (PBD_PROBE_ENV("PBD_DEBUG_SKIP_Y")) { hipMemsetAsync(d_sdt, 0, HW * ts, h->stream); hipMemsetAsync(d_iy, 0, HW * 2, h->stream); }
  else launch_dt_pass(d_tasks + nx, (int)tasks.size() - nx, d_maps, nullptr, nullptr, h->d_biasw, budget, tsz, nt, 0, h->stream);
  std::vector<int16_t> hx(HW), hy(HW);
  HIPCHK(h, hipMemcpyAsync(out, d_sdt, HW * ts, hipMemcpyDeviceToHost, h->stream));
  HIPCHK(h, hipMemcpyAsync(hx.data(), d_ixT, HW * 2, hipMemcpyDeviceToHost, h->stream));
  HIPCHK(h, hipMemcpyAsync(hy.data(), d_iy, HW * 2, hipMemcpyDeviceToHost, h->stream));
  std::vector<char> htmp(HW * ts);
  HIPCHK(h, hipMemcpyAsync(htmp.data(), d_tmp, HW * ts, hipMemcpyDeviceToHost, h->stream));
  HIPCHK(h, hipStreamSynchronize(h->stream));
  const bool left_domain = tsz == 4 ? pbd_first_nonfinite((const float*)htmp.data(), HW) != HW || pbd_first_nonfinite((const float*)out, HW) != HW
                                    : pbd_first_nonfinite((const double*)htmp.data(), HW) != HW || pbd_first_nonfinite((const double*)out, HW) != HW;
  for (size_t i = 0; i < HW; ++i) {
    const int m_ = (int)(i / cols), n_ = (int)(i - (size_t)m_ * cols);
    int x, y;
    if (!h->opt.dt_correct_ptr) { x = hx[(size_t)n_ * rows + m_]; y = hy[(size_t)m_ * cols + x]; }
    else { y = hy[i]; x = hx[(size_t)n_ * rows + y]; }
    if (ix) ix[i] = x;
    if (iy) iy[i] = y;
  }
  hipFree(d_in); hipFree(d_tmp); hipFree(d_sdt); hipFree(d_ixT); hipFree(d_iy);
  hipFree(d_maps); hipFree(d_tasks);
  if (left_domain)
    return fail(h, PBD_ERR_ARG, "the scores left the finite range in the x or the y pass (|y| + |a| d^2 + |b| d overflows): outside the distance transform's domain");
  return PBD_OK;
}
int pbd_dt2d(pbd_handle* h, const float* in, int rows, int cols, double ax, double bx, double ay, double by, int osx,
             int osy, float* out, int32_t* ix, int32_t* iy) {
  return dt2d_(h, in, rows, cols, ax, bx, ay, by, osx, osy, out, ix, iy, 4);
}
int pbd_dt2d_f64(pbd_handle* h, const double* in, int rows, int cols, double ax, double bx, double ay, double by, int osx,
                 int osy, double* out, int32_t* ix, int32_t* iy) {
  return dt2d_(h, in, rows, cols, ax, bx, ay, by, osx, osy, out, ix, iy, 8);
}

static int hog_u8_(pbd_handle* h, const uint8_t* im, int w, int hgt, int cn, int stride, void* out, int* cell_w, int* cell_h, int ts) {
  if (!h || !im || w < 3 || hgt < 3 || (cn != 1 && cn != 3) || stride < w * cn) return PBD_ERR_ARG;
  CHECK_SCALAR(h, ts);
  ON_DEVICE(h);
  const int sbin = h->md.sbin;
  LevelDev L{};
  L.iw = w; L.ih = hgt;
  L.bw = (int)std::round((float)w / (float)sbin); L.bh = (int)std::round((float)hgt / (float)sbin);
  L.cw = std::max(L.bw - 2, 0); L.ch = std::max(L.bh - 2, 0);
  if (cell_w) *cell_w = L.cw;
  if (cell_h) *cell_h = L.ch;
  if (L.cw == 0 || L.ch == 0) return PBD_OK;
  int tc = 16;
  while (tc > 2 && hog_lds_bytes(sbin, tc, ts) > 150 * 1024) tc /= 2;
  std::vector<HogTile> tiles;
  for (int y = 0; y < L.ch; y += tc) for (int x = 0; x < L.cw; x += tc) tiles.push_back(HogTile{0, y, x, 0});
  uint8_t* d_im; char* d_feat; LevelDev* d_lv; HogTile* d_tiles;
  HIPCHK(h, hipMalloc(&d_im, (size_t)w * hgt * cn)); HIPCHK(h, hipMalloc(&d_feat, (size_t)L.cw * L.ch * PBD_FLEN * ts));
  HIPCHK(h, hipMalloc(&d_lv, sizeof(L))); HIPCHK(h, hipMalloc(&d_tiles, sizeof(HogTile) * tiles.size()));
  HIPCHK(h, hipMemcpy2D(d_im, (size_t)w * cn, im, stride, (size_t)w * cn, hgt, hipMemcpyHostToDevice));
  HIPCHK(h, hipMemcpy(d_lv, &L, sizeof(L), hipMemcpyHostToDevice));
  HIPCHK(h, hipMemcpy(d_tiles, tiles.data(), sizeof(HogTile) * tiles.size(), hipMemcpyHostToDevice));
  launch_hog(d_tiles, (int)tiles.size(), d_lv, d_im, d_feat, ts, cn, sbin, tc, h->d_hog_lut, nullptr, 0, PBD_DEPTH_8U, h->stream);
  HIPCHK(h, hipStreamSynchronize(h->stream));
  HIPCHK(h, hipMemcpy(out, d_feat, (size_t)L.cw * L.ch * PBD_FLEN * ts, hipMemcpyDeviceToHost));
  hipFree(d_im); hipFree(d_feat); hipFree(d_lv); hipFree(d_tiles);
  return PBD_OK;
}
int pbd_hog_u8(pbd_handle* h, const uint8_t* im, int w, int hgt, int cn, int stride, float* out, int* cell_w, int* cell_h) {
  return hog_u8_(h, im, w, hgt, cn, stride, out, cell_w, cell_h, 4);
}
int pbd_hog_u8_f64(pbd_handle* h, const uint8_t* im, int w, int hgt, int cn, int stride, double* out, int* cell_w, int* cell_h) {
  return hog_u8_(h, im, w, hgt, cn, stride, out, cell_w, cell_h, 8);
}

int pbd_resize_u8(pbd_handle* h, const uint8_t* im, int w, int hgt, int cn, int stride, uint8_t* out, int ow, int oh) {
  if (!h || !im || !out || w <= 0 || hgt <= 0 || ow <= 0 || oh <= 0 || (cn != 1 && cn != 3) || stride < w * cn) return PBD_ERR_ARG;
  ON_DEVICE(h);
  uint8_t *d_im, *d_out;
  HIPCHK(h, hipMalloc(&d_im, (size_t)w * hgt * cn)); HIPCHK(h, hipMalloc(&d_out, (size_t)ow * oh * cn));
  HIPCHK(h, hipMemcpy2D(d_im, (size_t)w * cn, im, stride, (size_t)w * cn, hgt, hipMemcpyHostToDevice));
  PyrJob job{0, 0, w, hgt, ow, oh}, *d_job;
  HIPCHK(h, hipMalloc(&d_job, sizeof(job)));
  HIPCHK(h, hipMemcpy(d_job, &job, sizeof(job), hipMemcpyHostToDevice));
  launch_resize(d_job, 1, ow * oh, cn, w * cn, d_im, d_out, h->stream);
  HIPCHK(h, hipStreamSynchronize(h->stream));
  HIPCHK(h, hipMemcpy(out, d_out, (size_t)ow * oh * cn, hipMemcpyDeviceToHost));
  hipFree(d_im); hipFree(d_out); hipFree(d_job);
  return PBD_OK;
}

int pbd_pyrdown_u8(pbd_handle* h, const uint8_t* im, int w, int hgt, int cn, int stride, uint8_t* out) {
  if (!h || !im || !out || w <= 0 || hgt <= 0 || (cn != 1 && cn != 3) || stride < w * cn) return PBD_ERR_ARG;
  ON_DEVICE(h);
  const size_t sb = (size_t)w * hgt * cn, db = (size_t)((w + 1) / 2) * ((hgt + 1) / 2) * cn;
  uint8_t* d_buf;
  HIPCHK(h, hipMalloc(&d_buf, sb + db));
  HIPCHK(h, hipMemcpy2D(d_buf, (size_t)w * cn, im, stride, (size_t)w * cn, hgt, hipMemcpyHostToDevice));
  PyrJob job{0, (unsigned long long)sb, w, hgt, (w + 1) / 2, (hgt + 1) / 2}, *d_job;
  HIPCHK(h, hipMalloc(&d_job, sizeof(job)));
  HIPCHK(h, hipMemcpy(d_job, &job, sizeof(job), hipMemcpyHostToDevice));
  launch_pyrdown(d_job, 1, job.dw, job.dh, cn, d_buf, h->stream);
  HIPCHK(h, hipStreamSynchronize(h->stream));
  HIPCHK(h, hipMemcpy(out, d_buf + sb, db, hipMemcpyDeviceToHost));
  hipFree(d_buf); hipFree(d_job);
// ... 126 lines not shown
```

### partsbaseddetector_amd/csrc/pbd_internal.hpp

```cpp
#pragma once
#include <hip/hip_runtime.h>
#include <stdint.h>
#include <string.h>
#include <string>
#include <vector>
#include "../../include/pbd_c.h"

#include "pbd_plan.hpp"
#include "pbd_lds.hpp"

#ifndef PBD_ARGMIN_ZERO_COPY
#define PBD_ARGMIN_ZERO_COPY 1
#endif
#ifndef PBD_DT_PRIO
#define PBD_DT_PRIO 1
#endif
#ifndef PBD_DT_TASK_PREFETCH
#define PBD_DT_TASK_PREFETCH 256
#endif

struct CandRec { int level, comp, y, x; };

struct LatJob {
  void* plane;
// ... 21 lines not shown
struct LatentSource { const int32_t* truth; const int32_t* mix; int component; double overlap; };

struct RecordSet {
  const char* p; size_t stride; int mp;
  const int* count; int capacity;
  const int* cf; int nframes;
  int nlevels;
};
struct DepthFrames {
  const char* img; size_t pitch, fbytes; int w, h; unsigned long long has;
};
#ifdef __HIPCC__
__device__ __forceinline__ int record_frame(const RecordSet& r, int i) {
  if (r.cf) {
    for (int k = 0; k < r.nframes; ++k)
      if (i >= r.cf[2 + r.nframes + k] && i < r.cf[2 + r.nframes + k] + r.cf[2 + k]) return k;
    return -1;
  }
  return r.nlevels ? ((const pbd_candidate_head*)(r.p + r.stride * (size_t)i))->level / r.nlevels : 0;
}
#endif

struct Cl3Res { pbd_cluster3d r; long long off; };

struct Cluster3dArgs {
  RecordSet in;
  DepthFrames z; size_t pstride;
  const int* list; int nlist;
  const pbd_box3d* boxes;
  pbd_camera cam;
  float tol;
  char* scratch; size_t slot_bytes; int pcap;
  Cl3Res* out;
  int* pool; unsigned long long pool_cap; unsigned long long* pool_used;
};

struct pbd_handle : HostModel {
  std::vector<char> level_set;
  std::string err;
  PlanKnobs knobs;

  void* d_wT = nullptr;
  int ncu = 256;
  int nfpad = 0;
  float* d_biasw = nullptr;
  uint8_t* d_hog_lut = nullptr;
  int* d_parent = nullptr;
  int* d_plane0 = nullptr;
  int* d_nparts = nullptr;
  int* d_mix_rows = nullptr;

  int fw = 0, fh = 0, fcn = 0, nlevels = 0;
  int dt_geom = 0;
  int fdepth = 0, fesz = 1;
  int ldepth = 0, lesz = 1;
  int batch = 1, nvl = 0;
  std::vector<Level> lv;
  PyrJob* d_pyrjobs = nullptr;
  std::vector<PyrLaunch> pyr_launches;
  MatJob* d_matjobs = nullptr; MatRun* d_matruns = nullptr; MatTap* d_mattaps = nullptr;
  size_t cells = 0, pyr_bytes = 0;
  bool have_pyr = false, have_feat = false, have_resp = false, have_dp = false;
  std::vector<char> feat_ok, resp_ok;
  bool min_ran = false;
  bool ik_lazy = false;
  std::vector<char> ext_set, root_set;

  uint8_t* d_img = nullptr; size_t img_cap = 0;
  uint8_t* d_pyr = nullptr;
  char* d_feat = nullptr; char* d_resp = nullptr; char* d_acc = nullptr;
  uint16_t* d_feat_split = nullptr;
  bool feat_split_ok = false;
  float* d_split_oscale = nullptr;
  uint16_t* d_wS = nullptr;
  uint8_t* d_pk = nullptr;
  unsigned long long* d_scr_base = nullptr;
  unsigned long long* d_pick = nullptr;
  ReduceBlock* d_ik_blocks = nullptr; unsigned* d_ik_cells = nullptr; int n_ik_blocks = 0;
  std::vector<unsigned long long> scr_base;
  int* d_flat = nullptr;
  int* d_depth = nullptr;
  int max_depth = 0;
  char* d_rootv = nullptr; int* d_rooti = nullptr;
  char* d_dt_tmpT = nullptr; char* d_dt_sdt = nullptr; int16_t* d_dt_ixT = nullptr; int16_t* d_dt_iy = nullptr;
  size_t dt_cap_elems = 0;
  LevelDev* d_levels = nullptr;
  LevelDev* d_hog_levels = nullptr;
  PadJob* d_padjobs = nullptr; ReduceBlock* d_padblocks = nullptr; int n_padblocks = 0;
  HogTile* d_hog_tiles = nullptr; int n_hog_tiles = 0; int hog_tc = 16;
  ConvTile* d_conv_tiles = nullptr; int n_conv_tiles = 0;
  ConvTile* d_conv_tiles_mix = nullptr;
  DtMap* d_dtmaps = nullptr; DtTask* d_dttasks = nullptr;
  ReduceJob* d_redjobs = nullptr; ReduceBlock* d_redblocks = nullptr; RootJob* d_rootjobs = nullptr; BackLevel* d_back = nullptr;
  size_t dt_lds = 0;
  bool compact = false;
  FoldJob* d_foldjobs = nullptr;
  unsigned long long* d_foldx = nullptr;
  int dt_nt = PBD_DT_NT_DEFAULT;
  std::vector<RoundLaunch> rl;
  int n_rootjobs = 0; unsigned root_cells = 0, root_maxcells = 0;
  uint8_t* d_nms_mask = nullptr;
  ReduceBlock* d_rootblocks = nullptr; int n_rootblocks = 0;
  int* d_cand_count = nullptr; CandRec* d_cand_rec = nullptr;
  char* d_cand_out = nullptr; char* h_cand_out = nullptr; int* h_cand_count = nullptr;
  bool out_on_host = false;
  size_t cand_stride = 0;
  bool pending = false;
  int first_copy = 0;
  char* d_gsend = nullptr;

  hipStream_t stream = nullptr;
  bool own_stream = false;
  bool profiling = false;
  hipEvent_t ev[8] = {};
  float stage_ms[6] = {0, 0, 0, 0, 0, 0};
  hipEvent_t ev_dp0 = nullptr, ev_dp1 = nullptr;
  double dp_ms_sum = 0; int dp_frames = 0; bool dp_timer_on = true; bool dp_timed = false;
  hipGraphExec_t gexec = nullptr;
  int frames_on_plan = 0;
  std::vector<void*> frame_allocs;
  struct ModelBuf { void* p; size_t bytes; bool pinned; };
  std::vector<ModelBuf> model_allocs;
  size_t frame_bytes = 0, model_bytes = 0;
  int16_t* d_extx = nullptr; int16_t* d_exty = nullptr; unsigned long long* d_ext_base = nullptr;
  bool ext_ptr = false;
  bool root_dirty = false;
  int cand_mode = PBD_CAND_RAW; float cand_overlap = 0.f;
  bool in_group = false;
  bool cand_defer = false;
  bool out_filtered = false;
  char* d_cand_raw = nullptr;
  unsigned long long* d_cf_keys = nullptr; unsigned* d_cf_idx = nullptr; int* d_cf_box = nullptr; uint8_t* d_cf_st = nullptr;
  int* d_cf_cnt = nullptr; int* h_cf_cnt = nullptr;
  unsigned long long* d_cf_mask = nullptr; size_t cf_mask_bytes = 0;
  int cand_nms = PBD_NMS_PAINTED; int cand_top = 0;
  char* d_cp_stage = nullptr; int* d_cp_cnt = nullptr;
  int4* d_cp_rect = nullptr; int* d_cp_np = nullptr; unsigned* d_cp_kept = nullptr; unsigned long long* d_cp_bits = nullptr;
  bool zf_on = false; float zf_factor = 0.f;
  bool zf_frame = false;
  const char* zf_img = nullptr; size_t zf_pitch = 0, zf_fbytes = 0; unsigned long long zf_has = 0;
  int* d_zf_npart = nullptr; int* d_zf_par = nullptr; double* d_zf_thr = nullptr; float zf_thr_factor = 0.f;
  unsigned long long* d_zf_med = nullptr; unsigned* d_zf_large = nullptr;
  int* d_zf_cnt = nullptr;
  char* d_zf_out = nullptr;
  char* d_zimg = nullptr; size_t zimg_bytes = 0;
  bool b3_on = false; pbd_camera b3_cam{};
  bool b3_frame = false;
  unsigned long long b3_has = 0;
  pbd_box3d* h_b3 = nullptr; double* h_b3c = nullptr;
  bool b3_ready = false;
  std::vector<std::vector<pbd_box3d>> b3_res; std::vector<std::vector<double>> b3_cen; std::vector<char> b3_res_on;
  bool cl3_on = false; float cl3_tol = 0.01f;
  bool cl3_frame = false;
  Cl3Res* h_cl3 = nullptr;
  char* d_cl3_scratch = nullptr; int cl3_slots = 0, cl3_pcap = 0;
  int* d_cl3_pool = nullptr; unsigned long long cl3_pool_cap = 0; unsigned long long* d_cl3_used = nullptr;
  Cluster3dArgs cl3_args{};
  bool cl3_ready = false;
  std::vector<std::vector<int>> cl3_slot;
  std::vector<std::vector<pbd_cluster3d>> cl3_res; std::vector<std::vector<int32_t>> cl3_idx; std::vector<char> cl3_res_on;
  bool ps_on = false;
  bool ps_frame = false;
  bool ps_compact = false;
  struct PsMix* d_ps_mix = nullptr; int* d_ps_mix0 = nullptr;
  double* h_ps = nullptr;
  bool ps_ready = false;
  std::vector<std::vector<double>> ps_res; std::vector<char> ps_res_on;
// ... 136 lines not shown
int pbd_i_post_buffers(pbd_handle* h);
int pbd_i_post_enqueue(pbd_handle* h, int cm, bool zf, char* raw);
int pbd_i_run_box3d(pbd_handle* h);
int pbd_i_run_part_scores(pbd_handle* h);
void pbd_i_ps_begin(pbd_handle* h, int nframes);
void pbd_i_ps_gather(pbd_handle* h, int f, const std::vector<const char*>& recs, const std::vector<int>& order);
void pbd_i_b3_begin(pbd_handle* h, int nframes);
void pbd_i_b3_gather(pbd_handle* h, int f, const std::vector<const char*>& recs, const std::vector<int>& order);
int pbd_i_b3_end(pbd_handle* h);
int pbd_i_filter_host(pbd_handle* h, int mode, float overlap, int im_w, int im_h, char* recs, int count, int* kept,
                      int kind = PBD_NMS_PAINTED, int top = 0);
int pbd_i_depth_check(pbd_handle* h, int depth_type, long long dstride, int w);
template <typename T>
int dev_alloc(pbd_handle* h, T** p, size_t n) {
  void* q = nullptr;
  hipError_t e = hipMalloc(&q, (n > 1 ? n : 1) * sizeof(T));
  if (e != hipSuccess) { h->err = std::string("hipMalloc: ") + hipGetErrorString(e); return PBD_ERR_HIP; }
  h->frame_allocs.push_back(q);
  h->frame_bytes += (n > 1 ? n : 1) * sizeof(T);
  *p = (T*)q;
  return PBD_OK;
}
template <typename T>
int model_alloc(pbd_handle* h, T** p, size_t n, bool pinned = false, bool counted = true) {
  void* q = nullptr;
  hipError_t e = pinned ? hipHostMalloc(&q, sizeof(T) * n) : hipMalloc(&q, sizeof(T) * n);
  if (e != hipSuccess) return fail(h, PBD_ERR_HIP, std::string(pinned ? "hipHostMalloc: " : "hipMalloc: ") + hipGetErrorString(e));
  h->model_allocs.push_back({q, counted ? sizeof(T) * n : 0, pinned});
  h->model_bytes += h->model_allocs.back().bytes;
  *p = (T*)q;
  return PBD_OK;
}
inline void model_free(pbd_handle* h, void* p) {
  for (auto b = h->model_allocs.begin(); b != h->model_allocs.end(); ++b)
    if (b->p == p) { if (b->pinned) hipHostFree(p); else hipFree(p); h->model_bytes -= b->bytes; h->model_allocs.erase(b); return; }
}
template <typename T, typename C>
int model_grow(pbd_handle* h, T** p, C& have, C need, size_t n = 0) {
  if (need <= have) return PBD_OK;
  if (*p) { model_free(h, *p); *p = nullptr; }
  have = 0;
  int rc = model_alloc(h, p, n ? n : (size_t)need);
  if (!rc) have = need;
  return rc;
}

void launch_resize(const PyrJob* jobs, int njobs, int maxpix, int cn, int sstride, const uint8_t* src, uint8_t* pyr, hipStream_t s);
void launch_pyrdown(const PyrJob* jobs, int njobs, int maxw, int maxh, int cn, uint8_t* pyr, hipStream_t s);
void launch_hog(const HogTile* tiles, int ntiles, const LevelDev* levels, const uint8_t* pyr, void* feat, int ts,
                int cn, int sbin, int tc, const uint8_t* binlut, uint16_t* split, int split_parts, int depth, hipStream_t s);
void launch_resize_area(const MatJob* jobs, int njobs, int maxpix, const MatRun* runs, const MatTap* taps, int cn, int sstride,
                        bool src_f64, const uint8_t* src, uint8_t* pyr, hipStream_t s);
void launch_reduce_f64(const MatJob* jobs, int njobs, int maxpix, int cn, uint8_t* pyr, hipStream_t s);
void launch_resize_any(const PyrJob* jobs, int njobs, int maxpix, int cn, int depth, int sstride, const uint8_t* src, uint8_t* pyr, hipStream_t s);
void launch_pyrdown_any(const PyrJob* jobs, int njobs, int maxpix, int cn, int depth, uint8_t* pyr, hipStream_t s);
void launch_featpad(const PadJob* jobs, const ReduceBlock* blocks, int nblocks, void* feat, int ts, uint16_t* split, int split_parts, hipStream_t s);
size_t hog_binlut_bytes();
void launch_hog_binlut(uint8_t* lut, int ts, hipStream_t s);
void launch_feat_split(const float* feat, uint16_t* out, size_t ncells, hipStream_t s);
void launch_conv_split(const ConvTile* tiles, int ntiles, const LevelDev* levels, const uint16_t* feat_split, const uint16_t* wS,
                       float* resp, int nf, int kh, int kw, hipStream_t s, int nf_stride = 0);
void conv_split_filters(const float* filters, int nf, int kh, int kw, std::vector<uint16_t>& out);
void launch_feat_split16(const float* feat, uint16_t* out, size_t ncells, hipStream_t s);
void conv_split16_filters(const float* filters, int nf, int kh, int kw, std::vector<uint16_t>& out, std::vector<float>& oscale);
void launch_conv_split16(const ConvTile* tiles, int ntiles, const LevelDev* levels, const uint16_t* feat_split, const uint16_t* wS,
                         float* resp, int nf, int kh, int kw, const float* oscale, hipStream_t s, int nf_stride = 0);
void launch_conv_exact(const ConvTile* tiles, int ntiles, const LevelDev* levels, const void* feat,
                       const void* wT, void* resp, int ts, int nf, int nfpad, int kh, int kw, hipStream_t s, int nf_stride = 0);
void launch_conv_mfma_f64(const ConvTile* tiles, int ntiles, const LevelDev* levels, const double* feat,
                          const double* w4u, double* resp, int nf, int nfpad, int kh, int kw, hipStream_t s, int nf_stride = 0);
void launch_conv_mfma16_f32(const ConvTile* tiles, int ntiles, const LevelDev* levels, const float* feat,
                            const float* w4u, float* resp, int nf, int nfpad, int kh, int kw, hipStream_t s, int nf_stride = 0);
void launch_dt_pass(const DtTask* tasks, int ntasks, const DtMap* maps, const FoldJob* folds, const unsigned long long* foldx, const float* biasw, size_t lds,
                    int ts, int nt, int fm, hipStream_t s);
void launch_reduce(const ReduceJob* jobs, const ReduceBlock* blocks, int nblocks, const float* biasw, int correct_ptr,
                   int ts, hipStream_t s);
void launch_root(const RootJob* jobs, const ReduceBlock* blocks, int nblocks, double thresh, int* count, CandRec* rec,
                 int capacity, int ts, const FoldJob* folds, const float* biasw, int rescan, int fm, const uint8_t* nms_mask,
                 const char* rootv_base, hipStream_t s);
void launch_nms_roots(const RootJob* jobs, int njobs, unsigned maxcells, const char* rootv_base, int ts, int sz, uint8_t* mask, hipStream_t s);
void launch_backtrack(const int* count, const CandRec* rec, int capacity, const BackLevel* back, int ncomp,
                      const int* parent, const int* plane0, const int* nparts, int max_parts, const int* mix_rows,
                      char* out, size_t out_stride, int ts, const int* flat, const int* depth, int max_depth, int nflat,
                      const unsigned long long* scr_base, const int16_t* ix, const int16_t* iy, int correct_ptr,
                      const int16_t* extx, const int16_t* exty, const unsigned long long* ext_base, int* count_out, int pad,
                      const FoldJob* folds, const unsigned long long* pick, hipStream_t s);
void launch_ik_fill(const FoldJob* folds, const unsigned long long* pick, const ReduceBlock* blocks, int nblocks, const unsigned* cells, int ts, hipStream_t s);
void launch_latent_mask(const LatentMaskArgs& a, int nblocks, int ts, hipStream_t s);
void launch_latent_best(const LatentBestArgs& a, int ts, hipStream_t s);
void dt_debug_read(unsigned long long* out);
void dt_debug_counters(unsigned long long* out);
int dt_debug_trace(unsigned long long* t, unsigned* hw, int* nlaunch);
void hog_debug_read(unsigned long long* out);
void conv_debug_read(unsigned long long* out);
void launch_nms_map(const float* src, int rows, int cols, int sz, uint8_t* dst, hipStream_t s);
struct CandFilterArgs {
  RecordSet in;
  const BackLevel* back;
  const char* rootv_base; int ts, ncomp;
  int nms; double overlap; int im_w, im_h;
  unsigned long long* keys; unsigned* idx;
  int* box; unsigned char* st;
  unsigned long long* gmask;
  char* out; int* cnt_out;
};
size_t cand_filter_mask_bytes(int w, int h);
void launch_cand_filter(const CandFilterArgs& a, int nframes, hipStream_t s);
struct CandPartsArgs {
  const char* in; size_t stride; int mp;
  const int* cnt_in; int capacity;
  double overlap; int top;
  int4* rect;
  int* np; unsigned* kept;
  unsigned long long* gbits;
  char* out; int* cnt_out;
};
size_t cand_parts_bits_words(int capacity, int nframes);
void launch_cand_parts(const CandPartsArgs& a, int nframes, hipStream_t s);
struct ZFilterArgs {
  RecordSet in;
  DepthFrames z;
  const int* npart; const int* par; const double* thr;
  unsigned long long* med;
  unsigned* large; unsigned* nlarge;
  char* out; int* cnt;
  unsigned char* flags;
};
void launch_zfilter(const ZFilterArgs& a, int ts, hipStream_t s);
#define PBD_B3_MAXTAPS 35
struct Box3dArgs {
  RecordSet in;
  DepthFrames z;
  int im_w, im_h;
  pbd_camera cam;
  int ntaps; int tap_off[PBD_B3_MAXTAPS]; float tap[PBD_B3_MAXTAPS];
  pbd_box3d* out; double* centres;
};
void launch_box3d(const Box3dArgs& a, int ts, hipStream_t s);
struct PsMix { int filter, bias, ax, ay; float w[4]; };
struct PartScoreArgs {
  RecordSet in;
  const LevelDev* levels; int nvl;
  const char* resp; int nfilters;
  int ncomp, nbias;
  const int* nparts; const int* parent; const int* flat;
  const int* mix0; const PsMix* mix;
  const float* biasw;
  double* out;
};
void launch_partscore(const PartScoreArgs& a, int ts, hipStream_t s);
struct FvMix { int def, filter, kh, kw; };
struct FeatVecArgs {
  RecordSet in;
  int rec0, n;
  const LevelDev* levels; int nvl;
  const char* feat;
  int ncomp, nbias, nfilters;
  const int* nparts; const int* parent; const int* flat;
  const int* mix0; const PsMix* mix; const FvMix* fmix;
  int wmax;
  pbd_feature_block* blocks;
  void* windows;
};
void launch_featvec(const FeatVecArgs& a, int ts, hipStream_t s);
size_t cluster3d_slot_bytes(int pcap);
void launch_cluster3d(const Cluster3dArgs& a, int src, int nblocks, hipStream_t s);
```

### partsbaseddetector_amd/csrc/pbd_plan.cpp

```cpp
#include "pbd_plan.hpp"
#include <algorithm>
#include <cmath>
#include <cstdlib>
#include <map>
#include "dt_core.hpp"
#include "pbd_lds.hpp"

static int fail(std::string* err, int code, const std::string& msg) {
  if (err) *err = msg;
  return code;
}

static inline int cv_round_f(float v) { return (int)std::lrint((double)v); }

int compute_geometry(int w, int h, int sbin, int interval, int* nlevels, Level* lv) {
  const float sf = (float)std::pow(2.0, (double)(1.0f / (float)interval));
  const float fw = (float)w, fh = (float)h;
  const float mn = fh < fw ? fh : fw;
  const float r = std::log(mn / (5.0f * (float)sbin)) / std::log(sf);
  const int n = (int)(1.0f + std::floor(r));
  if (n < interval || n > PBD_MAX_LEVELS) return -1;
  for (int i = 0; i < interval; ++i) {
    const float f = (float)(1.0f / std::pow((double)sf, (double)i));
    lv[i].iw = cv_round_f(fw * f);
// ... 243 lines not shown
  return PBD_OK;
}

int plan_model(HostModel& hm, const pbd_model_desc* model, const int32_t* fsize, bool sized, const pbd_options* opt, std::string* err) {
  HostModel* h = &hm;
  pbd_options o{};
  if (opt) o = *opt;
  if (o.max_candidates <= 0) o.max_candidates = 4096;
  h->opt = o;
  if (o.scalar_type != PBD_SCALAR_F32 && o.scalar_type != PBD_SCALAR_F64) return fail(err, PBD_ERR_ARG, "scalar_type: PBD_SCALAR_F32 or PBD_SCALAR_F64");
  h->ts = (o.scalar_type == PBD_SCALAR_F64) ? 8 : 4;
  pbd_model_desc sdesc;
  std::vector<float> sorted;
  if (sized && !fsize) return fail(err, PBD_ERR_ARG, "pbd_create_sized: fsize is null");
  if (sized) {
    if (!model || !model->filters) return fail(err, PBD_ERR_ARG, "model: null pointer");
    if (model->kh != 0 || model->kw != 0) return fail(err, PBD_ERR_ARG, "pbd_create_sized: model->kh / kw must be 0 (the sizes come from fsize)");
    if (model->nfilters <= 0) return fail(err, PBD_ERR_ARG, "model: bad sizes");
    if (model->flen != PBD_FLEN || model->norient != PBD_NORIENT)
      return fail(err, PBD_ERR_UNSUPPORTED, "model: only flen=32 / norient=18 HOG is supported");
    const int nf = model->nfilters;
    for (int n = 0; n < nf; ++n)
      if (fsize[2 * n] < 1 || fsize[2 * n] > 9 || fsize[2 * n + 1] < 1 || fsize[2 * n + 1] > 9)
        return fail(err, PBD_ERR_UNSUPPORTED, "pbd_create_sized: filter " + std::to_string(n) + ": sides of 1..9 cells");
    sdesc = *model;
    bool uniform = true;
    for (int n = 1; n < nf; ++n) uniform = uniform && fsize[2 * n] == fsize[0] && fsize[2 * n + 1] == fsize[1];
    if (uniform) {
      sdesc.kh = fsize[0]; sdesc.kw = fsize[1];
    } else {
      std::vector<int> ord(nf);
      for (int n = 0; n < nf; ++n) ord[n] = n;
      std::stable_sort(ord.begin(), ord.end(), [&](int a, int b) {
        return fsize[2 * a] != fsize[2 * b] ? fsize[2 * a] < fsize[2 * b] : fsize[2 * a + 1] < fsize[2 * b + 1]; });
      std::vector<size_t> off(nf + 1, 0);
      for (int n = 0; n < nf; ++n) off[n + 1] = off[n] + (size_t)fsize[2 * n] * fsize[2 * n + 1] * PBD_FLEN;
      h->mixed = true;
      h->fperm.assign(nf, 0);
      for (int i = 0; i < nf; ++i) {
        const int c = ord[i];
        h->fperm[c] = i;
        h->fkh.push_back(fsize[2 * c]); h->fkw.push_back(fsize[2 * c + 1]);
        sorted.insert(sorted.end(), model->filters + off[c], model->filters + off[c + 1]);
      }
      sdesc.filters = sorted.data();
    }
    model = &sdesc;
  }
  int rc = ingest_model(h, model, err);
  if (rc) return rc;
  if (h->mixed) {
    for (int& f : h->filterid) f = h->fperm[f];
    for (PartInfo& P : h->parts) for (int& f : P.filterid) f = h->fperm[f];
  }
  if (o.reserved[0] < 0 || o.reserved[0] > 1024) return fail(err, PBD_ERR_ARG, "reserved[0] (nms_sz): 0 = off, or the window of the score-map NMS");
  h->nms_sz = o.reserved[0];
  h->conv_mode = o.conv_mode;
  if (h->conv_mode == PBD_CONV_AUTO)
    {
      bool splittable = h->ts == 4 && model->flen == PBD_FLEN;
      for (size_t i = 0; splittable && i < h->filters.size(); ++i) splittable = std::fabs(h->filters[i]) < 3.0e38f;
      h->conv_mode = model->nfilters >= 16 ? (splittable ? PBD_CONV_SPLIT : PBD_CONV_MFMA) : PBD_CONV_EXACT;
    }
  if ((h->conv_mode == PBD_CONV_SPLIT || h->conv_mode == PBD_CONV_SPLIT_F16) && (h->ts != 4 || model->flen != PBD_FLEN))
    return fail(err, PBD_ERR_UNSUPPORTED, "PBD_CONV_SPLIT / PBD_CONV_SPLIT_F16: float handles (32-channel HOG features)");
  if (h->conv_mode == PBD_CONV_SPLIT || h->conv_mode == PBD_CONV_SPLIT_F16)
    for (size_t i = 0; i < h->filters.size(); ++i)
      if (!(std::fabs(h->filters[i]) < 3.0e38f)) return fail(err, PBD_ERR_UNSUPPORTED, "PBD_CONV_SPLIT: a filter weight outside bfloat16's finite range");
  if (h->conv_mode < PBD_CONV_AUTO || h->conv_mode > PBD_CONV_SPLIT_F16) return fail(err, PBD_ERR_ARG, "conv_mode: PBD_CONV_*");
  if (h->mixed)
    for (int n = 0; n < model->nfilters;) {
      int e = n;
      while (e < model->nfilters && h->fkh[e] == h->fkh[n] && h->fkw[e] == h->fkw[n]) ++e;
      SizeGroup g;
      g.kh = h->fkh[n]; g.kw = h->fkw[n]; g.n0 = n; g.nf = e - n;
      h->groups.push_back(g);
      n = e;
    }
  h->split_parts = h->conv_mode == PBD_CONV_SPLIT ? 3 : h->conv_mode == PBD_CONV_SPLIT_F16 ? 2 : 0;
  return PBD_OK;
}

static bool has_cells(const Level& L) { return L.active && L.cw > 0 && L.ch > 0; }

int plan_layout(const HostModel& hm, const FrameSpec& f, FrameLayout& out, std::string* err) {
  const pbd_model_desc& m = hm.md;
  out = FrameLayout{};
  int n1 = 0;
  std::vector<Level> lv((size_t)PBD_MAX_LEVELS, Level{});
  const bool matlab = hm.pyr_kind == PBD_PYRAMID_MATLAB;
  if (matlab && f.depth != PBD_DEPTH_8U)
    return fail(err, PBD_ERR_UNSUPPORTED, "PBD_PYRAMID_MATLAB: 8-bit frames (the level images are double whatever the frame; pbd_set_pyramid_kind)");
  if (matlab) {
    if (f.w < 3 || f.h < 3 || compute_geometry_matlab(f.w, f.h, m.sbin, m.interval, &n1, lv.data()))
      return fail(err, PBD_ERR_ARG, "image too small: the pyramid needs at least `interval` levels and reduce() sources of 5 x 5 pixels "
                                    "(matlab/detection/featpyramid.m:15, matlab/mex/reduce.cc:24-42)");
  } else
  if (f.w < 3 || f.h < 3 || compute_geometry(f.w, f.h, m.sbin, m.interval, &n1, lv.data()))
    return fail(err, PBD_ERR_ARG, "image too small: the pyramid needs at least `interval` levels "
                                  "(src/HOGFeatures.cpp:99,114)");
  pad_geometry(hm.pad, n1, lv.data());
  const int n = n1 * f.batch;
  out.nlevels = n1; out.batch = f.batch; out.nvl = n;
  out.src_esz = depth_esz(f.depth);
  out.esz = matlab ? 8 : out.src_esz;
  out.lv.resize(n);
  for (int fr = 0; fr < f.batch; ++fr)
    for (int l = 0; l < n1; ++l) out.lv[fr * n1 + l] = lv[l];
  int lb = hm.opt.level_begin, le = hm.opt.level_end;
  if (le <= 0 || le > n1) le = n1;
  if (lb < 0) lb = 0;
  size_t cells = 0, pyr = 0;
  for (int vl = 0; vl < n; ++vl) {
    Level& L = out.lv[vl];
    const int l = vl % n1;
    L.active = (l >= lb && l < le) && (f.level_set.empty() || (l < (int)f.level_set.size() && f.level_set[l]));
    if (L.cw > 32767 || L.ch > 32767) return fail(err, PBD_ERR_UNSUPPORTED, "level too large for 16-bit pointers");
    if ((size_t)L.cw * L.ch >= ((size_t)1 << 28)) return fail(err, PBD_ERR_UNSUPPORTED, "level too large (2^28 cells)");
    L.img_off = pyr; pyr += (size_t)L.iw * L.ih * f.cn * out.esz;
    L.cell_off = cells; cells += (size_t)L.cw * L.ch;
    if (L.active) out.act_cells += (size_t)L.cw * L.ch;
  }
  out.cells = cells; out.pyr_bytes = pyr;
  if (matlab && pyr > PBD_MATPYR_MAX_BYTES)
    return fail(err, PBD_ERR_UNSUPPORTED, "PBD_PYRAMID_MATLAB: the double level images of this geometry exceed the plan's budget for them (2 GiB)");
  if (cells >= (1u << 31)) return fail(err, PBD_ERR_UNSUPPORTED, "frame too large");
  for (const std::vector<int>& rnd : hm.rounds) {
    size_t k = 0;
    for (int fp : rnd) k += hm.parts[fp].K;
    out.maxK = std::max(out.maxK, k);
  }
  size_t allmaps = 0;
  for (const PartInfo& P : hm.parts) if (P.p > 0) allmaps += P.K;
  out.dt_cap_elems = std::max<size_t>(1, allmaps * out.act_cells);

  const size_t ts = (size_t)hm.ts;
  out.compact = hm.fold && hm.unique_filters && (hm.opt.reserved[1] == 2 || (hm.opt.reserved[1] == 0 && cells * m.nfilters * ts > ((size_t)400 << 20)));
  auto own = [&](FrameBuf b, size_t bytes) {
    out.buf[b] = BufPlace{(int)out.regions.size(), 0, std::max<size_t>(bytes, 1)};
    out.regions.push_back(out.buf[b].bytes);
  };
  own(FB_IMG, (size_t)f.w * f.h * f.cn * out.src_esz * f.batch);
  own(FB_RESP, cells * m.nfilters * ts);
  const size_t pk_bytes = cells * std::max(hm.nplanes, 1), feat_bytes = cells * PBD_FLEN * ts;
  const size_t tmp_elems = hm.fold ? std::max<size_t>(1, out.maxK * out.act_cells) : out.dt_cap_elems;
  if (out.compact) {
    const size_t al = 256, pyr_al = (pyr + al - 1) / al * al, pk_al = (pk_bytes + al - 1) / al * al;
    const int r = (int)out.regions.size();
    out.regions.push_back(std::max<size_t>(1, std::max(pyr_al + feat_bytes, pk_al + out.maxK * out.act_cells * ts)));
    out.buf[FB_PYR] = BufPlace{r, 0, pyr};
    out.buf[FB_FEAT] = BufPlace{r, pyr_al, feat_bytes};
    out.buf[FB_PK] = BufPlace{r, 0, pk_bytes};
    out.buf[FB_DT_TMPT] = BufPlace{r, pk_al, out.maxK * out.act_cells * ts};
  } else {
    own(FB_PYR, pyr);
    own(FB_FEAT, feat_bytes);
    own(FB_PK, pk_bytes);
    own(FB_DT_TMPT, tmp_elems * ts);
    own(FB_DT_SDT, out.dt_cap_elems * ts);
  }
  own(FB_ROOTV, cells * m.ncomponents * ts);
  own(FB_ROOTI, std::max<size_t>(cells * m.ncomponents, 1) * sizeof(int));
  if (hm.nms_sz > 0) own(FB_NMS_MASK, cells * m.ncomponents);
  own(FB_DT_IXT, out.dt_cap_elems * sizeof(int16_t));
  own(FB_DT_IY, out.dt_cap_elems * sizeof(int16_t));
  if (!hm.fold) own(FB_ACC, cells * hm.nslots * ts);
  if (hm.split_parts) {
    const size_t split_elems = cells * hm.split_parts * PBD_FLEN;
    if (out.compact && out.dt_cap_elems >= split_elems) out.buf[FB_FEAT_SPLIT] = BufPlace{out.buf[FB_DT_IXT].region, 0, split_elems * sizeof(uint16_t)};
    else own(FB_FEAT_SPLIT, split_elems * sizeof(uint16_t));
  }
  return PBD_OK;
}

FrameBases frame_bases(const FrameLayout& lay, char* const* regions) {
  FrameBases b{};
  for (int i = 0; i < FB_COUNT; ++i)
    b.p[i] = lay.buf[i].region < 0 ? nullptr : regions[lay.buf[i].region] + lay.buf[i].offset;
  return b;
}

int dt_stride_for(int len) { return (len + 1) | 1; }
static int dt_lpb_for(int stride, int len, int unit, size_t budget, int ts, int nt, int seg, bool round_lanes) {
  const int lmin = unit > 1 ? unit : 4;
  int lpb = std::min(nt, 128);
  if (unit > 1) lpb = std::max(unit, lpb / unit * unit);
  while (lpb > lmin && dt_lds_bytes(stride, lpb, ts, nt) > budget) lpb -= (unit > 1 ? unit : 1);
  if (round_lanes && unit <= 1 && lpb > lmin) lpb = std::max(lmin, nt / ((nt + lpb - 1) / lpb));
  if (seg > 0) {
    const int P = std::max(1, std::min(nt / 4, (len + seg - 1) / seg));
    int cap = std::max(lmin, nt / P);
    if (unit > 1) cap = std::max(unit, cap / unit * unit);
    lpb = std::min(lpb, cap);
  }
  return lpb;
}
DtGroup dt_group(int map0, int nmaps, int nlines, int len, size_t budget, int ts, int nt, int seg, bool natural, int fold, bool round_lanes) {
  DtGroup g{};
  g.map0 = map0; g.nmaps = nmaps; g.nlines = nlines; g.len = len; g.fold = fold;
  g.fused = natural ? DT_G_NATURAL : 0;
  g.stride = dt_stride_for(len);
  g.lpb = dt_lpb_for(g.stride, len, fold >= 0 ? nmaps : 1, budget, ts, nt, seg, round_lanes);
  g.nsub = nt / g.lpb;
  g.P = dt_segments(g.nsub, len);
  g.chunk = (len + g.nsub - 1) / g.nsub;
  g.magic_lpb = dt_magic((unsigned)g.lpb);
  g.magic_nlines = dt_magic((unsigned)nlines);
  g.magic_P = dt_magic((unsigned)g.P);
  return g;
}
void dt_add_tasks(const DtGroup& g, std::vector<DtTask>& out, const std::vector<DtMap>* maps, int ts) {
  if (g.fold >= 0) {
    const int R = g.lpb / g.nmaps;
    for (int r0 = 0; r0 < g.nlines; r0 += R) out.push_back(DtTask{r0, std::min(R, g.nlines - r0) * g.nmaps, 0, r0, g, nullptr});
  } else {
    const int total = g.nmaps * g.nlines;
    const size_t map_bytes = (size_t)g.nlines * g.len * ts;
    for (int g0 = 0; g0 < total; g0 += g.lpb) {
      DtTask t{g0, std::min(g.lpb, total - g0), g0 / g.nlines, g0 % g.nlines, g, nullptr};
      if (maps && g.len > 1) {
        const int mlast = (g0 + t.nl - 1) / g.nlines;
        bool contig = true;
        for (int m = t.m0; m < mlast && contig; ++m)
          contig = (const char*)(*maps)[(size_t)g.map0 + m + 1].src == (const char*)(*maps)[(size_t)g.map0 + m].src + map_bytes;
        if (contig) t.src0 = (const char*)(*maps)[(size_t)g.map0 + t.m0].src + (size_t)t.l0 * g.len * ts;
      }
      out.push_back(t);
    }
  }
}
void dt_mark_fused(std::vector<DtTask>& tasks, const DtMap* maps, int ts) {
  for (DtTask& t : tasks) {
    DtGroup& g = t.g;
    bool ok = ts == 4 && g.len <= DT_FUSE_MAXLEN;
    for (int m = 0; m < g.nmaps && ok; ++m) {
      const DtMap& mp = maps[g.map0 + m];
      ok = (double)(float)mp.a == mp.a && (double)(float)mp.b == mp.b && (long long)g.len + std::abs((long long)mp.os) <= DT_FUSE_MAXLEN;
    }
    if (ok) g.fused |= DT_G_FUSED;
  }
}
DtMap dt_map(const void* src, void* dst, int16_t* ptr, float wq, float wl, int os, int natural) {
  DtMap m{};
  m.src = src; m.dst = dst; m.ptr = ptr;
  m.a = -(double)wq; m.b = -(double)wl;
  m.r2a = 1.0 / (2.0 * m.a);
  m.os = os; m.ptr_natural = natural;
  return m;
}

static void pyramid_jobs(const HostModel& hm, const FrameSpec& f, const FrameLayout& lay, FrameTables& out) {
  const int n1 = lay.nlevels, interval = hm.md.interval;
  std::vector<PyrJob>& jobs = out.pyrjobs;
  PyrLaunch R{0, 0, 1, 1, 1};
  for (int fr = 0; fr < f.batch; ++fr)
    for (int i = 0; i < interval; ++i) {
      const Level& L = lay.lv[fr * n1 + i];
      jobs.push_back(PyrJob{(unsigned long long)fr * f.w * f.h * f.cn * lay.src_esz, (unsigned long long)L.img_off, f.w, f.h, L.iw, L.ih});
      R.maxpix = std::max(R.maxpix, L.iw * L.ih);
    }
  R.njobs = (int)jobs.size();
  out.pyr_launches.push_back(R);
  for (int base = interval; base < n1; base += interval) {
    PyrLaunch D{(int)jobs.size(), 0, 1, 1, 1};
    for (int fr = 0; fr < f.batch; ++fr)
      for (int j = base; j < std::min(base + interval, n1); ++j) {
        const Level &S = lay.lv[fr * n1 + j - interval], &L = lay.lv[fr * n1 + j];
        jobs.push_back(PyrJob{(unsigned long long)S.img_off, (unsigned long long)L.img_off, S.iw, S.ih, L.iw, L.ih});
        D.maxpix = std::max(D.maxpix, L.iw * L.ih);
        D.maxw = std::max(D.maxw, L.iw); D.maxh = std::max(D.maxh, L.ih);
      }
    D.njobs = (int)jobs.size() - D.job0;
    out.pyr_launches.push_back(D);
  }
}

static bool pyramid_jobs_matlab(const HostModel& hm, const FrameSpec& f, const FrameLayout& lay, FrameTables& out) {
  const int n1 = lay.nlevels, interval = hm.md.interval;
  std::vector<MatJob>& jobs = out.matjobs;
  std::vector<int> yrun0((size_t)interval), xrun0((size_t)interval);
  for (int i = 0; i < interval; ++i) {
    const Level& L = lay.lv[i];
    yrun0[i] = (int)out.matruns.size();
    if (!resize_taps(f.h, L.ih, out.matruns, out.mattaps)) return false;
    xrun0[i] = (int)out.matruns.size();
    if (!resize_taps(f.w, L.iw, out.matruns, out.mattaps)) return false;
  }
  PyrLaunch R{0, 0, 1, 1, 1};
  for (int fr = 0; fr < f.batch; ++fr)
    for (int i = 0; i < interval; ++i) {
      const Level& L = lay.lv[fr * n1 + i];
      jobs.push_back(MatJob{(unsigned long long)fr * f.w * f.h * f.cn * lay.src_esz, (unsigned long long)L.img_off, f.w, f.h, L.iw, L.ih, yrun0[i], xrun0[i]});
      R.maxpix = std::max(R.maxpix, L.iw * L.ih);
    }
  R.njobs = (int)jobs.size();
  out.pyr_launches.push_back(R);
  for (int base = interval; base < n1; base += interval) {
    PyrLaunch D{(int)jobs.size(), 0, 1, 1, 1};
    for (int fr = 0; fr < f.batch; ++fr)
      for (int j = base; j < std::min(base + interval, n1); ++j) {
        const Level &S = lay.lv[fr * n1 + j - interval], &L = lay.lv[fr * n1 + j];
        jobs.push_back(MatJob{(unsigned long long)S.img_off, (unsigned long long)L.img_off, S.iw, S.ih, L.iw, L.ih, 0, 0});
        D.maxpix = std::max(D.maxpix, L.iw * L.ih);
        D.maxw = std::max(D.maxw, L.iw); D.maxh = std::max(D.maxh, L.ih);
      }
    D.njobs = (int)jobs.size() - D.job0;
    out.pyr_launches.push_back(D);
  }
  return true;
}

static int hog_conv_tiles(const HostModel& hm, const FrameSpec& f, const FrameLayout& lay, FrameTables& out, std::string* err) {
  const int sbin = hm.md.sbin;
  const int hog_bpp = lay.esz == 1 ? 3 : f.cn * lay.esz;
  out.hog_tc = 16;
  while (out.hog_tc > 2 && hog_lds_bytes(sbin, out.hog_tc, hm.ts, hog_bpp) > 150 * 1024) out.hog_tc /= 2;
  if (hog_lds_bytes(sbin, out.hog_tc, hm.ts, hog_bpp) > 150 * 1024) return fail(err, PBD_ERR_UNSUPPORTED, "sbin too large");
  std::vector<ConvTile> ct;
  for (int l = 0; l < lay.nvl; ++l) {
    const Level& L = lay.lv[l];
    if (!has_cells(L)) continue;
    for (int y = 0; y < L.ch - 2 * hm.pad; y += out.hog_tc)
      for (int x = 0; x < L.cw - 2 * hm.pad; x += out.hog_tc) out.hog_tiles.push_back(HogTile{l, y, x, 0});
    for (int y = 0; y < L.ch; y += 16)
      for (int x = 0; x < L.cw; x += 16) ct.push_back(ConvTile{l, y, x, 0});
  }
  out.conv_tiles = ct;
  const size_t full = ct.size() / 16 * 16;
  for (size_t b = 0; b < full; b += 16)
    for (size_t x = 0; x < 8; ++x) { out.conv_tiles[b + x] = ct[b + 2 * x]; out.conv_tiles[b + 8 + x] = ct[b + 2 * x + 1]; }
  if (hm.mixed)
    for (const SizeGroup& g : hm.groups)
      for (ConvTile t : out.conv_tiles) { t.pad = g.n0 | (g.nf << 16); out.conv_tiles_mix.push_back(t); }
  return PBD_OK;
}

static int dt_geometry(const HostModel& hm, const FrameLayout& lay, int dt_geom, const PlanKnobs& kn, FrameTables& out, std::string* err) {
  int maxlen = 1;
  for (const Level& L : lay.lv) if (L.active) maxlen = std::max(maxlen, std::max(L.cw, L.ch));
  const bool byte_links = dt_stride_for(maxlen) <= 256;
  const bool big_blocks = hm.ts == 4 && dt_geom ? dt_geom == 1 : byte_links;
  out.dt_nt = hm.ts == 8 ? 128 : (big_blocks ? 256 : PBD_DT_NT_DEFAULT);
  if (kn.dt_nt) out.dt_nt = kn.dt_nt;
  size_t dt_base = (hm.ts == 8 ? 40 : (big_blocks ? 40 : 25)) * 1024;
  if (kn.dt_budget_kb >= 0) dt_base = (size_t)kn.dt_budget_kb * 1024;
  if (kn.dt_budget_b >= 0) dt_base = (size_t)kn.dt_budget_b;
  int max_mix = 4;
  if (hm.fold) for (const PartInfo& P : hm.parts) max_mix = std::max(max_mix, P.K);
  const size_t dt_need = dt_lds_bytes(dt_stride_for(maxlen), max_mix, hm.ts, out.dt_nt);
  if (dt_need > 160 * 1024) return fail(err, PBD_ERR_UNSUPPORTED, "pyramid level too large for the LDS-resident distance transform");
  out.dt_lds = std::max(dt_base, dt_need);
  return PBD_OK;
}

struct PlaneAddr {
  const HostModel& hm;
  const FrameLayout& lay;
  const FrameBases& b;
  std::vector<size_t> part_scr, lvl_scr;
  PlaneAddr(const HostModel& hm_, const FrameLayout& lay_, const FrameBases& b_) : hm(hm_), lay(lay_), b(b_), part_scr(hm_.parts.size(), 0), lvl_scr(lay_.nvl, 0) {
    size_t o = 0;
    for (size_t fp = 0; fp < hm.parts.size(); ++fp) if (hm.parts[fp].p > 0) { part_scr[fp] = o; o += (size_t)hm.parts[fp].K * lay.act_cells; }
    o = 0;
    for (int l = 0; l < lay.nvl; ++l) { lvl_scr[l] = o; if (lay.lv[l].active) o += (size_t)lay.lv[l].cw * lay.lv[l].ch; }
  }
  size_t hw(int l) const { return (size_t)lay.lv[l].cw * lay.lv[l].ch; }
  size_t scr_of(int fp, int l, int mm) const { return part_scr[fp] + (size_t)hm.parts[fp].K * lvl_scr[l] + (size_t)mm * hw(l); }
  char* resp(int l, int fid) const { return b.p[FB_RESP] + (lay.lv[l].cell_off * hm.md.nfilters + (size_t)fid * hw(l)) * hm.ts; }
  char* acc(int l, int slot) const { return b.p[FB_ACC] + (lay.lv[l].cell_off * hm.nslots + (size_t)slot * hw(l)) * hm.ts; }
  char* sdt(int fp, int l, int mm) const { return lay.compact ? resp(l, hm.parts[fp].filterid[mm]) : b.p[FB_DT_SDT] + scr_of(fp, l, mm) * hm.ts; }
  uint8_t* ik(int l, int plane0) const { return (uint8_t*)b.p[FB_PK] + lay.lv[l].cell_off * hm.nplanes + (size_t)plane0 * hw(l); }
};

static int make_fold(const HostModel& hm, const PlaneAddr& pa, const std::vector<int>& children, int fp, int l, FrameTables& out) {
  if (children.empty()) return -1;
  std::vector<FoldJob>& folds = out.folds;
  FoldJob J{};
  for (int c : children) {
    const PartInfo& C = hm.parts[c];
    out.pick[(size_t)l * hm.parts.size() + c] = folds.size() * sizeof(FoldJob) + offsetof(FoldJob, ch) + (size_t)J.nch * sizeof(FoldChild);
    FoldChild& F = J.ch[J.nch++];
    F.K = C.K; F.L = hm.parts[fp].K;
    for (int k = 0; k < PBD_FOLD_MAXMIX; ++k) F.sdt[k] = pa.sdt(c, l, std::min(k, C.K - 1));
    const int Lp = hm.parts[fp].K;
    for (int k = 0; k < PBD_FOLD_MAXMIX; ++k)
      for (int mm = 0; mm < PBD_FOLD_MAXMIX; ++mm)
        F.bias[k][mm] = hm.biasw[C.biasid[std::min(k, C.K - 1)] + std::min(mm, Lp - 1)];
    F.ok = pa.ik(l, C.plane0);
  }
  folds.push_back(J);
  return (int)folds.size() - 1;
}

struct Geo { size_t budget; bool round; };
static Geo launch_geometry(const HostModel& hm, const FrameLayout& lay, const std::vector<int>& rnd, size_t base, bool fold_x, bool ypass,
                           int nt, int seg, int ncu) {
  if (fold_x) return Geo{base, true};
  int nm = 0;
  for (int fp : rnd) nm += hm.parts[fp].K;
  const int waves_blk = std::max(1, nt / 64);
  auto resident = [&](size_t budget, bool round_lanes) {
    size_t nb = 0, lds = 0;
    for (const Level& L : lay.lv) {
      if (!has_cells(L)) continue;
      const int len = ypass ? L.ch : L.cw, nlines = ypass ? L.cw : L.ch;
      const DtGroup g = dt_group(0, nm, nlines, len, budget, hm.ts, nt, seg, !ypass, -1, round_lanes);
      nb += ((size_t)nm * nlines + g.lpb - 1) / g.lpb;
      lds = std::max(lds, dt_lds_bytes(g.stride, g.lpb, hm.ts, nt));
    }
    const size_t per_cu = std::min<size_t>(160 * 1024 / std::max<size_t>(lds, 1), 24 / waves_blk);
    return nb <= per_cu * ncu;
  };
  if (resident(base, true)) return Geo{base, true};
  if (resident(base, false)) return Geo{base, false};
  for (size_t b = base + 1024; b <= base * 8 / 5 && b <= 150 * 1024; b += 1024) {
    if (resident(b, true)) return Geo{b, true};
    if (resident(b, false)) return Geo{b, false};
  }
  return Geo{base, true};
}

static void xcd_order(std::vector<DtTask>& v, int c) {
  if (c <= 0) return;
  const size_t win = (size_t)8 * c, full = v.size() / win * win;
  std::vector<DtTask> o(v);
  for (size_t b = 0; b < full; ++b) {
    const size_t xcd = b & 7, idx = b >> 3;
    o[b] = v[((idx / c) * 8 + xcd) * c + idx % c];
  }
  v.swap(o);
}
static size_t launch_lds(const std::vector<DtTask>& v, int ts, int nt) {
  size_t lds = 0;
  for (const DtTask& t : v) lds = std::max(lds, dt_lds_bytes(t.g.stride, t.g.lpb, ts, nt));
  return lds;
}

static void dt_round(const HostModel& hm, const FrameLayout& lay, const PlaneAddr& pa, const std::vector<std::vector<int>>& children,
                     size_t r, int ncu, const PlanKnobs& kn, const std::vector<char>& slot_init, FrameTables& out, RoundLaunch& R) {
  const std::vector<int>& rnd = hm.rounds[r];
  const bool fold = hm.fold, fold_x = fold && r > 0;
  const int ts = hm.ts, nt = out.dt_nt, seg = kn.dt_seg;
  const Geo geox = launch_geometry(hm, lay, rnd, out.dt_lds, fold_x, false, nt, seg, ncu);
  const Geo geoy = launch_geometry(hm, lay, rnd, out.dt_lds, false, true, nt, seg, ncu);
  size_t roundK = 0;
  for (int fp : rnd) roundK += hm.parts[fp].K;
  std::vector<DtMap>& maps = out.maps;
  std::vector<DtTask> xt, yt;
  for (int l = 0; l < lay.nvl; ++l) {
    const Level& L = lay.lv[l];
    if (!has_cells(L)) continue;
    const size_t HW = (size_t)L.cw * L.ch;
    const int gx_map0 = (int)maps.size();
    int gx_nmaps = 0;
    std::vector<DtMap> ymaps;
    size_t tmp_round = 0;
    for (int fp : rnd) {
      const PartInfo& P = hm.parts[fp];
      const int part_map0 = (int)maps.size();
      for (int mm = 0; mm < P.K; ++mm) {
        const int fid = P.filterid[mm], did = P.defid[mm];
        const size_t so = pa.scr_of(fp, l, mm);
        const size_t to = fold ? roundK * pa.lvl_scr[l] + (tmp_round + (size_t)mm) * HW : so;
        const char* src = (!fold && slot_init[P.slot[mm]]) ? pa.acc(l, P.slot[mm]) : pa.resp(l, fid);
        const float* wv = &hm.defw[(size_t)did * 4];
        char* tmp = pa.b.p[FB_DT_TMPT] + to * ts;
        maps.push_back(dt_map(src, tmp, (int16_t*)pa.b.p[FB_DT_IXT] + so, wv[0], wv[1], hm.anchors[did * 2], 1));
        ymaps.push_back(dt_map(tmp, pa.sdt(fp, l, mm), (int16_t*)pa.b.p[FB_DT_IY] + so, wv[2], wv[3], hm.anchors[did * 2 + 1], 0));
        gx_nmaps++;
      }
      tmp_round += (size_t)P.K;
      if (fold_x) dt_add_tasks(dt_group(part_map0, P.K, L.ch, L.cw, geox.budget, ts, nt, seg, true, make_fold(hm, pa, children[fp], fp, l, out)), xt);
    }
    if (!fold_x) dt_add_tasks(dt_group(gx_map0, gx_nmaps, L.ch, L.cw, geox.budget, ts, nt, seg, true, -1, geox.round), xt, &maps, ts);
    const DtGroup gy = dt_group((int)maps.size(), gx_nmaps, L.cw, L.ch, geoy.budget, ts, nt, seg, false, -1, geoy.round);
    for (auto& my : ymaps) maps.push_back(my);
    dt_add_tasks(gy, yt, &maps, ts);
  }
  dt_mark_fused(xt, maps.data(), ts);
  dt_mark_fused(yt, maps.data(), ts);
  xcd_order(xt, kn.xcd_chunk);
  xcd_order(yt, kn.xcd_chunk);
  R.lds_x = launch_lds(xt, ts, nt); R.lds_y = launch_lds(yt, ts, nt); R.fold_x = fold_x ? 1 : 0;
  if (fold_x) {
    R.foldx0 = out.foldx.size();
    for (const DtTask& t : xt) {
      const DtGroup& g = t.g;
      for (int mm = 0; mm < 8; ++mm) out.foldx.push_back((unsigned long long)(uintptr_t)maps[(size_t)g.map0 + std::min(mm, g.nmaps - 1)].src);
      const unsigned long long* cq = (const unsigned long long*)&out.folds[(size_t)g.fold].ch[0];
      for (int i = 0; i < 9; ++i) out.foldx.push_back(cq[i]);
      out.foldx.push_back((unsigned long long)out.folds[(size_t)g.fold].nch);
    }
  }
  R.xtask0 = (int)out.tasks.size(); R.nxtasks = (int)xt.size();
  out.tasks.insert(out.tasks.end(), xt.begin(), xt.end());
  R.ytask0 = (int)out.tasks.size(); R.nytasks = (int)yt.size();
  out.tasks.insert(out.tasks.end(), yt.begin(), yt.end());
}

static void reduce_waves(const HostModel& hm, const FrameLayout& lay, const PlaneAddr& pa, size_t r, std::vector<char>& slot_init,
                         FrameTables& out, RoundLaunch& R) {
  for (const std::vector<int>& wave : hm.red_rounds[r]) {
    ReduceWave Wv{(int)out.redblk.size(), 0};
    std::vector<int> parents;
    for (int fp : wave) {
      const int pf = hm.part_offset[hm.parts[fp].comp] + hm.parts[fp].parent;
      if (std::find(parents.begin(), parents.end(), pf) == parents.end()) parents.push_back(pf);
    }
    for (int l = 0; l < lay.nvl; ++l) {
      const Level& L = lay.lv[l];
      if (!has_cells(L)) continue;
      const size_t HW = (size_t)L.cw * L.ch;
      for (int pf : parents) {
        const PartInfo& Par = hm.parts[pf];
        ReduceJob J{};
        J.H = L.ch; J.W = L.cw; J.L = Par.K;
        for (int pm = 0; pm < Par.K; ++pm) {
          char* accp = pa.acc(l, Par.slot[pm]);
          J.par_in[pm] = slot_init[Par.slot[pm]] ? accp : pa.resp(l, Par.filterid[pm]);
          J.par_out[pm] = accp;
        }
        for (int fp : wave) {
          const PartInfo& P = hm.parts[fp];
          if (hm.part_offset[P.comp] + P.parent != pf) continue;
          ReduceChild& C = J.ch[J.nch++];
          C.sdt = pa.sdt(fp, l, 0);
          C.ok = pa.ik(l, P.plane0);
          C.K = P.K;
          for (int mm = 0; mm < P.K; ++mm) C.bias_off[mm] = P.biasid[mm];
        }
        for (unsigned c0 = 0; c0 < (unsigned)HW; c0 += 256) out.redblk.push_back(ReduceBlock{(int)out.red.size(), c0});
        out.red.push_back(J);
      }
    }
    for (int pf : parents)
      for (int pm = 0; pm < hm.parts[pf].K; ++pm) slot_init[hm.parts[pf].slot[pm]] = 1;
    Wv.nblks = (int)out.redblk.size() - Wv.blk0;
    R.waves.push_back(Wv);
  }
}

static void root_tables(const HostModel& hm, const FrameLayout& lay, const PlaneAddr& pa, const std::vector<std::vector<int>>& children,
                        const std::vector<char>& slot_init, FrameTables& out) {
  const int nc = hm.md.ncomponents;
  const size_t ts = (size_t)hm.ts;
  out.back.assign((size_t)lay.nvl * nc, BackLevel{});
  for (int l = 0; l < lay.nvl; ++l) {
    const Level& L = lay.lv[l];
    const size_t HW = (size_t)L.cw * L.ch;
    for (int c = 0; c < nc; ++c) {
      BackLevel& B = out.back[(size_t)l * nc + c];
      B.pk = pa.ik(l, hm.comp_plane0[c]);
      B.rootv = pa.b.p[FB_ROOTV] + (L.cell_off * nc + (size_t)c * HW) * ts;
      B.rooti = (int*)pa.b.p[FB_ROOTI] + L.cell_off * nc + (size_t)c * HW;
      B.H = L.ch; B.W = L.cw; B.scale = L.scale;
      if (!L.active || HW == 0) continue;
      const PartInfo& R0 = hm.parts[hm.part_offset[c]];
      RootJob J{};
      for (int kk = 0; kk < PBD_MAX_MIX; ++kk) {
        const int k = std::min(kk, R0.K - 1);
        J.score[kk] = (!hm.fold && slot_init[R0.slot[k]]) ? pa.acc(l, R0.slot[k]) : pa.resp(l, R0.filterid[k]);
      }
      J.rootv = (void*)B.rootv; J.rooti = (int*)B.rooti;
// ... 56 lines not shown
```

### partsbaseddetector_amd/csrc/pbd_plan.hpp

```cpp
#pragma once
#include <cmath>
#include <stddef.h>
#include <stdint.h>
#include <string>
#include <vector>
#include "../../include/pbd_c.h"

#define PBD_MAX_LEVELS 128
#define PBD_FLEN 32
#define PBD_NORIENT 18
#define PBD_MAX_MIX 16

struct Level {
  int iw, ih;
  int bw, bh;
  int cw, ch;
  float scale;
  size_t img_off;
  size_t cell_off;
  int active;
};

struct PyrJob { unsigned long long soff, doff; int sw, sh, dw, dh; };
struct MatTap { double alpha; int si, pad; };
struct MatRun { int first, count; };
struct MatJob { unsigned long long soff, doff; int sw, sh, dw, dh, yrun0, xrun0; };
struct HogTile { int level, cy0, cx0, pad; };
struct LevelDev {
  int iw, ih, bw, bh, cw, ch;
  unsigned long long img_off, cell_off;
};
struct ConvTile { int level, y0, x0, pad; };
struct PadJob { unsigned long long cell_off; int cw, ch, pad, nring; };
#define PBD_FEATPAD_CPB 64

struct DtMap {
  const void* src;
  void* dst;
  int16_t* ptr;
  double a, b;
  double r2a;
  int os, ptr_natural;
};
struct DtGroup {
  int map0, nmaps, nlines, len, stride, lpb, fold;
  int nsub;
  int P;
  int chunk;
  unsigned magic_lpb;
  unsigned magic_nlines;
  unsigned magic_P;
  int fused;
};
#define DT_G_FUSED 1
#define DT_G_NATURAL 2
struct DtTask { int g0, nl, m0, l0; DtGroup g;
  const void* src0; };
static inline unsigned dt_magic(unsigned d) { return d > 1 ? 0xFFFFFFFFu / d + 1u : 0u; }
#define PBD_MAX_CH 8
struct ReduceChild {
  const void* sdt;
  uint8_t* ok;
  int K, pad;
  int bias_off[PBD_MAX_MIX];
};
#define PBD_FOLDX_QW 18
#define PBD_FOLD_MAXMIX 8
struct FoldChild {
  const void* sdt[PBD_FOLD_MAXMIX];
  uint8_t* ok;
  int K, L;
  float bias[PBD_FOLD_MAXMIX][PBD_FOLD_MAXMIX];
};
struct FoldJob { int nch, pad; FoldChild ch[PBD_MAX_CH]; };
#define PBD_NO_PICK (~0ull)
struct ReduceJob {
  int H, W, L, nch;
  const void* par_in[PBD_MAX_MIX];
  void* par_out[PBD_MAX_MIX];
  ReduceChild ch[PBD_MAX_CH];
};
struct ReduceBlock { int job; unsigned cell0; };
struct RootJob {
  const void* score[PBD_MAX_MIX];
  void* rootv; int* rooti;
  int H, W, K, level, comp;
  float bias;
  unsigned cell0;
  int fold, pad;
};
struct BackLevel {
  const uint8_t* pk;
  const void* rootv; const int* rooti;
  int H, W; float scale;
};

static_assert(sizeof(Level) == 56, "Level layout");
static_assert(sizeof(PyrJob) == 32, "PyrJob layout");
static_assert(sizeof(MatTap) == 16 && sizeof(MatRun) == 8 && sizeof(MatJob) == 40, "MatTap / MatRun / MatJob layout");
static_assert(sizeof(HogTile) == 16, "HogTile layout");
static_assert(sizeof(LevelDev) == 40, "LevelDev layout");
static_assert(sizeof(ConvTile) == 16, "ConvTile layout");
static_assert(sizeof(PadJob) == 24, "PadJob layout");
static_assert(sizeof(DtMap) == 56, "DtMap layout");
static_assert(sizeof(DtGroup) == 56, "DtGroup layout");
static_assert(sizeof(DtTask) == 80, "DtTask layout");
static_assert(sizeof(FoldChild) == 336, "FoldChild layout");
static_assert(sizeof(FoldJob) == 2696, "FoldJob layout");
static_assert(sizeof(ReduceChild) == 88, "ReduceChild layout");
static_assert(sizeof(ReduceJob) == 976, "ReduceJob layout");
static_assert(sizeof(ReduceBlock) == 8, "ReduceBlock layout");
static_assert(sizeof(RootJob) == 184, "RootJob layout");
static_assert(sizeof(BackLevel) == 40, "BackLevel layout");

#ifndef PBD_DT_NT_DEFAULT
#define PBD_DT_NT_DEFAULT 128
#endif

struct PartInfo {
  int comp, p, parent;
  int K;
  std::vector<int> filterid, defid, biasid;
  std::vector<int> slot;
  int plane0;
  bool leaf;
};

struct SizeGroup {
  int kh = 0, kw = 0, n0 = 0, nf = 0, nfpad = 0;
  void* d_wT = nullptr; uint16_t* d_wS = nullptr; float* d_oscale = nullptr;
};


struct HostModel {
  pbd_model_desc md;
  std::vector<float> filters, defw, biasw;
  std::vector<int> anchors, part_offset, parentid, mix_offset, filterid, defid, biasid;
  pbd_options opt;
  int ts = 4;
  int conv_mode = PBD_CONV_EXACT;
  int split_parts = 0;
  int pad = 0;
  int pyr_kind = PBD_PYRAMID_OPENCV;
  int nms_sz = 0;
  int max_parts = 0, nslots = 0, nplanes = 0;
  std::vector<PartInfo> parts;
  std::vector<std::vector<int>> rounds;
  std::vector<std::vector<std::vector<int>>> red_rounds;
  std::vector<int> comp_plane0;
  bool unique_filters = false;
  bool fold = false;
  int fold_mix = 0;
  bool mixed = false;
  std::vector<int> fkh, fkw;
  std::vector<int> fperm;
  std::vector<SizeGroup> groups;
};
template <typename T>
static inline size_t pbd_first_nonfinite(const T* v, size_t n) {
  size_t i = 0;
  while (i < n && std::isfinite(v[i])) ++i;
  return i;
}
int plan_model(HostModel& hm, const pbd_model_desc* model, const int32_t* fsize, bool sized, const pbd_options* opt, std::string* err);

struct PlanKnobs {
  int dt_nt = 0;
  int dt_seg = 0;
  long long dt_budget_kb = -1;
  long long dt_budget_b = -1;
  int xcd_chunk = 16;
};

struct FrameSpec {
  int w = 0, h = 0, cn = 3, batch = 1, depth = PBD_DEPTH_8U;
  std::vector<char> level_set;
};
enum FrameBuf { FB_IMG, FB_PYR, FB_FEAT, FB_RESP, FB_PK, FB_ROOTV, FB_ROOTI, FB_NMS_MASK, FB_DT_TMPT, FB_DT_SDT, FB_DT_IXT, FB_DT_IY,
                FB_ACC, FB_FEAT_SPLIT, FB_COUNT };
struct BufPlace { int region = -1; size_t offset = 0, bytes = 0; };
struct FrameLayout {
  int nlevels = 0, batch = 1, nvl = 0, esz = 1;
  int src_esz = 1;
  std::vector<Level> lv;
  size_t cells = 0, pyr_bytes = 0;
  size_t act_cells = 0;
  size_t maxK = 1;
  size_t dt_cap_elems = 0;
  bool compact = false;
  BufPlace buf[FB_COUNT];
  std::vector<size_t> regions;
};
int plan_layout(const HostModel& hm, const FrameSpec& f, FrameLayout& out, std::string* err);

struct FrameBases { char* p[FB_COUNT]; };
FrameBases frame_bases(const FrameLayout& lay, char* const* regions);

struct PyrLaunch { int job0, njobs, maxpix, maxw, maxh; };
struct ReduceWave { int blk0, nblks; };
struct RoundLaunch { int xtask0, nxtasks, ytask0, nytasks; size_t lds_x, lds_y; int fold_x; std::vector<ReduceWave> waves;
                     size_t foldx0 = 0; };
struct FrameTables {
  std::vector<PyrJob> pyrjobs;
  std::vector<PyrLaunch> pyr_launches;
  std::vector<MatJob> matjobs;
  std::vector<MatRun> matruns;
  std::vector<MatTap> mattaps;
  std::vector<LevelDev> levels;
  std::vector<LevelDev> hog_levels;
  std::vector<PadJob> padjobs;
  std::vector<ReduceBlock> padblk;
  int hog_tc = 16;
  std::vector<HogTile> hog_tiles;
  std::vector<ConvTile> conv_tiles, conv_tiles_mix;
  int dt_nt = PBD_DT_NT_DEFAULT;
  size_t dt_lds = 0;
  std::vector<DtMap> maps;
  std::vector<DtTask> tasks;
  std::vector<FoldJob> folds;
  std::vector<unsigned long long> foldx;
  std::vector<ReduceJob> red;
  std::vector<ReduceBlock> redblk;
  std::vector<RoundLaunch> rl;
  std::vector<RootJob> rootjobs;
  std::vector<ReduceBlock> rootblk;
  std::vector<BackLevel> back;
  std::vector<unsigned long long> scr_base;
  std::vector<unsigned long long> pick;
  unsigned root_cells = 0, root_maxcells = 0;
};
int plan_tables(const HostModel& hm, const FrameSpec& f, const FrameLayout& lay, const FrameBases& b, int ncu, int dt_geom,
                const PlanKnobs& kn, FrameTables& out, std::string* err);

int dt_stride_for(int len);
DtGroup dt_group(int map0, int nmaps, int nlines, int len, size_t budget, int ts, int nt, int seg, bool natural, int fold = -1,
                 bool round_lanes = true);
void dt_add_tasks(const DtGroup& g, std::vector<DtTask>& out, const std::vector<DtMap>* maps = nullptr, int ts = 4);
void dt_mark_fused(std::vector<DtTask>& tasks, const DtMap* maps, int ts);
DtMap dt_map(const void* src, void* dst, int16_t* ptr, float wq, float wl, int os, int natural);

int compute_geometry(int w, int h, int sbin, int interval, int* nlevels, Level* lv);
int compute_geometry_matlab(int w, int h, int sbin, int interval, int* nlevels, Level* lv);
bool resize_taps(int slen, int dlen, std::vector<MatRun>& runs, std::vector<MatTap>& taps);
#define PBD_MATPYR_MAX_BYTES ((size_t)1 << 31)
void pad_geometry(int pad, int nlevels, Level* lv);
int depth_esz(int depth);
```

Measured before the change: 2411.

## Store DT argmax pointers as bytes and use fast max in fold children

When every distance-transform line fits in 256 positions, the argmax pointer planes (ixT/iy) are written and read as uint8 instead of int16, which halves the pointer write traffic in the DT pass and the reads in backtracking. Host readers and the planner are threaded with a ptr_bytes setting. Separately, the fold-children max over mixtures now uses a branchless fmax chain and falls back to the tie-aware fold_pick only when a wave ballot finds a zero or ambiguous result. Buffer allocation still sizes the pointer planes as int16, so they are over-allocated, and the fallback check adds a ballot per child.

```diff
diff --git a/partsbaseddetector_amd/csrc/fold_pick.hpp b/partsbaseddetector_amd/csrc/fold_pick.hpp
--- a/partsbaseddetector_amd/csrc/fold_pick.hpp
+++ b/partsbaseddetector_amd/csrc/fold_pick.hpp
@@ -26,3 +26,27 @@
   }
   return FoldPick<T>{K == 1 ? w0 : v, bi};
 }
+
+FP_HD float fold_maxnum(float a, float b) { return __builtin_fmaxf(a, b); }
+FP_HD double fold_maxnum(double a, double b) { return __builtin_fmax(a, b); }
+FP_HD float fold_abs(float a) { return __builtin_fabsf(a); }
+FP_HD double fold_abs(double a) { return __builtin_fabs(a); }
+
+template <typename T, int N = 0>
+FP_HD T fold_max_fast(const T* sd, const float* bias_col, int K) {
+  const int n = N > 0 ? N : K;
+  const T w0 = sd[0] + bias_col[0];
+  T v = fold_maxnum((T)-INFINITY, w0);
+#ifdef __HIPCC__
+#pragma unroll
+#endif
+  for (int k = 1; k < n; ++k) v = fold_maxnum(v, (T)(sd[k] + bias_col[k]));
+  return K == 1 ? w0 : v;
+}
+template <typename T> FP_HD bool fold_max_sure(T r) { return fold_abs(r) > (T)0; }
+
+template <typename T, int N = 0>
+FP_HD T fold_max(const T* sd, const float* bias_col, int K) {
+  const T r = fold_max_fast<T, N>(sd, bias_col, K);
+  return fold_max_sure(r) ? r : fold_pick<T, N>(sd, bias_col, K).v;
+}
diff --git a/partsbaseddetector_amd/csrc/k_dp.hip b/partsbaseddetector_amd/csrc/k_dp.hip
--- a/partsbaseddetector_amd/csrc/k_dp.hip
+++ b/partsbaseddetector_amd/csrc/k_dp.hip
@@ -62,6 +62,8 @@
   const unsigned lo = (unsigned)__builtin_amdgcn_readlane((int)(unsigned)v, l), hi = (unsigned)__builtin_amdgcn_readlane((int)(unsigned)(v >> 32), l);
   return (GP(char))(((unsigned long long)hi << 32) | lo);
 }
+__device__ __forceinline__ float fold_minnum(float a, float b) { return __builtin_fminf(a, b); }
+__device__ __forceinline__ double fold_minnum(double a, double b) { return __builtin_fmin(a, b); }
 template <typename T, int M, int U>
 __device__ __forceinline__ void fold_children(const FoldJob* __restrict__ J, const unsigned (&off)[U], T (&acc)[U][M], unsigned long long cv,
                                               int nch) {
@@ -93,11 +95,38 @@
 #pragma unroll
       for (int m = 0; m < M; ++m) bias[m][k] = C.bias[k][m];
     const int K = C.K;
-#pragma unroll
-    for (int u = 0; u < U; ++u)
-#pragma unroll
-      for (int m = 0; m < M; ++m)
-        acc[u][m] = acc[u][m] + fold_pick<T, M>(sd[u], bias[m], K).v;
+    if constexpr (sizeof(T) == 4 && M <= 6) {
+      T r[U][M];
+#pragma unroll
+      for (int u = 0; u < U; ++u)
+#pragma unroll
+        for (int m = 0; m < M; ++m) r[u][m] = fold_max_fast<T, M>(sd[u], bias[m], K);
+      T lo = fold_abs(r[0][0]);
+#pragma unroll
+      for (int i = 1; i < U * M; ++i) lo = fold_minnum(lo, fold_abs(r[i / M][i % M]));
+      if (__builtin_amdgcn_ballot_w64(!fold_max_sure(lo)) != 0) {
+#if defined(__HIP_DEVICE_COMPILE__)
+#pragma unroll
+        for (int u = 0; u < U; ++u)
+#pragma unroll
+          for (int k = 0; k < M; ++k) asm volatile("" : "+v"(sd[u][k]));
+#endif
+#pragma unroll
+        for (int u = 0; u < U; ++u)
+#pragma unroll
+          for (int m = 0; m < M; ++m) r[u][m] = fold_pick<T, M>(sd[u], bias[m], K).v;
+      }
+#pragma unroll
+      for (int u = 0; u < U; ++u)
+#pragma unroll
+        for (int m = 0; m < M; ++m) acc[u][m] = acc[u][m] + r[u][m];
+    } else {
+#pragma unroll
+      for (int u = 0; u < U; ++u)
+#pragma unroll
+        for (int m = 0; m < M; ++m)
+          acc[u][m] = acc[u][m] + fold_pick<T, M>(sd[u], bias[m], K).v;
+    }
   } while (++c < nch);
 }
 
@@ -325,7 +354,7 @@
 
   if (mine) {
     const double a = mp.a, b = mp.b;
-    int16_t* pp = mp.ptr + li;
+    const bool p8 = sizeof(IT) == 1 && (g.fused & DT_G_PTR8) != 0;
     const int chunk = g.chunk;
     const int q0 = p * chunk, q1 = min(len, q0 + chunk);
     if (q0 < q1) {
@@ -338,11 +367,13 @@
       int nnx = (int)Bl[nx];
       const int nlines = g.nlines;
       GPW(T) dp = (GPW(T))mp.dst + li + (size_t)(q1 - 1) * nlines;
-      GPW(int16_t) ppq = (GPW(int16_t))pp + (size_t)(q1 - 1) * nlines;
+      const size_t pe = (size_t)li + (size_t)(q1 - 1) * nlines;
       const int os_end = mp.os + q0;
       ++os;
-      auto outputs = [&](auto fused) {
+      auto outputs = [&](auto fused, auto ptype) {
         constexpr bool FZ = decltype(fused)::value;
+        typedef decltype(ptype) PT;
+        GPW(PT) ppq = (GPW(PT))mp.ptr + pe;
         do {
           --os;
           const T fos = (T)os;
@@ -350,12 +381,16 @@
           const double d = (double)(os - e);
           const double ad2 = a * (d * d);
           *dp = (T)((FZ ? fma(b, d, ad2) : (ad2 + b * d)) + (double)eyz.x);
-          *ppq = (int16_t)e;
+          *ppq = (PT)e;
           dp -= nlines; ppq -= nlines;
         } while (os > os_end);
       };
-      if constexpr (!EX) { if (fz) outputs(std::true_type{}); else outputs(std::false_type{}); }
-      else outputs(std::false_type{});
+      auto widths = [&](auto fused) {
+        if constexpr (sizeof(IT) == 1) { if (p8) { outputs(fused, (uint8_t)0); return; } }
+        outputs(fused, (int16_t)0);
+      };
+      if constexpr (!EX) { if (fz) widths(std::true_type{}); else widths(std::false_type{}); }
+      else widths(std::false_type{});
     }
   }
   DT_STAMP(5);
@@ -634,7 +669,7 @@
                                                   char* __restrict__ out, size_t out_stride,
                                                   const int* __restrict__ flat, const int* __restrict__ depth, int max_depth,
                                                   int nflat, const unsigned long long* __restrict__ scr_base,
-                                                  const int16_t* __restrict__ ixs, const int16_t* __restrict__ iys,
+                                                  const void* __restrict__ ixs, const void* __restrict__ iys, int ptr8,
                                                   int correct_ptr, const int16_t* __restrict__ extx,
                                                   const int16_t* __restrict__ exty, const unsigned long long* __restrict__ ext_base,
                                                   int* __restrict__ count_out, int org,
@@ -689,8 +724,9 @@
         x = extx[eo]; y = exty[eo];
       } else {
         const size_t so = (size_t)scr_base[(size_t)r.level * nflat + flat[r.comp * max_parts + p]] + (size_t)mm * HW;
-        if (!correct_ptr) { x = ixs[so + (size_t)px * B.H + py]; y = iys[so + (size_t)py * B.W + x]; }
-        else { y = iys[so + off]; x = ixs[so + (size_t)px * B.H + y]; }
+        auto at = [&](const void* pl, size_t i) { return ptr8 ? (int)((const uint8_t*)pl)[i] : (int)((const int16_t*)pl)[i]; };
+        if (!correct_ptr) { x = at(ixs, so + (size_t)px * B.H + py); y = at(iys, so + (size_t)py * B.W + x); }
+        else { y = at(iys, so + off); x = at(ixs, so + (size_t)px * B.H + y); }
       }
       lx[p] = x; ly[p] = y; lm[p] = mm;
     }
@@ -717,12 +753,12 @@
 void launch_backtrack(const int* count, const CandRec* rec, int capacity, const BackLevel* back, int ncomp,
                       const int* parent, const int* plane0, const int* nparts, int max_parts, const int* mix_rows, char* out,
                       size_t out_stride, int ts, const int* flat, const int* depth, int max_depth, int nflat,
-                      const unsigned long long* scr_base, const int16_t* ix, const int16_t* iy, int correct_ptr,
+                      const unsigned long long* scr_base, const void* ix, const void* iy, int ptr_bytes, int correct_ptr,
                       const int16_t* extx, const int16_t* exty, const unsigned long long* ext_base, int* count_out, int pad,
                       const FoldJob* folds, const unsigned long long* pick, hipStream_t s) {
   const int nblk = std::min(capacity, 2048);
-  if (ts == 8) hipLaunchKernelGGL(k_backtrack<double>, dim3(nblk), dim3(64), 0, s, count, rec, capacity, back, ncomp, parent, plane0, nparts, max_parts, mix_rows, out, out_stride, flat, depth, max_depth, nflat, scr_base, ix, iy, correct_ptr, extx, exty, ext_base, count_out, 1 + pad, (const char*)folds, pick);
-  else hipLaunchKernelGGL(k_backtrack<float>, dim3(nblk), dim3(64), 0, s, count, rec, capacity, back, ncomp, parent, plane0, nparts, max_parts, mix_rows, out, out_stride, flat, depth, max_depth, nflat, scr_base, ix, iy, correct_ptr, extx, exty, ext_base, count_out, 1 + pad, (const char*)folds, pick);
+  if (ts == 8) hipLaunchKernelGGL(k_backtrack<double>, dim3(nblk), dim3(64), 0, s, count, rec, capacity, back, ncomp, parent, plane0, nparts, max_parts, mix_rows, out, out_stride, flat, depth, max_depth, nflat, scr_base, ix, iy, ptr_bytes == 1, correct_ptr, extx, exty, ext_base, count_out, 1 + pad, (const char*)folds, pick);
+  else hipLaunchKernelGGL(k_backtrack<float>, dim3(nblk), dim3(64), 0, s, count, rec, capacity, back, ncomp, parent, plane0, nparts, max_parts, mix_rows, out, out_stride, flat, depth, max_depth, nflat, scr_base, ix, iy, ptr_bytes == 1, correct_ptr, extx, exty, ext_base, count_out, 1 + pad, (const char*)folds, pick);
 }
 
 template <typename T>
diff --git a/partsbaseddetector_amd/csrc/pbd_api.cpp b/partsbaseddetector_amd/csrc/pbd_api.cpp
--- a/partsbaseddetector_amd/csrc/pbd_api.cpp
+++ b/partsbaseddetector_amd/csrc/pbd_api.cpp
@@ -263,7 +263,7 @@
   h->cells = lay.cells; h->pyr_bytes = lay.pyr_bytes; h->compact = lay.compact; h->dt_cap_elems = lay.dt_cap_elems;
   h->d_img = (uint8_t*)b.p[FB_IMG]; h->d_pyr = (uint8_t*)b.p[FB_PYR]; h->d_feat = b.p[FB_FEAT]; h->d_resp = b.p[FB_RESP];
   h->d_pk = (uint8_t*)b.p[FB_PK]; h->d_rootv = b.p[FB_ROOTV]; h->d_rooti = (int*)b.p[FB_ROOTI]; h->d_nms_mask = (uint8_t*)b.p[FB_NMS_MASK];
-  h->d_dt_tmpT = b.p[FB_DT_TMPT]; h->d_dt_sdt = b.p[FB_DT_SDT]; h->d_dt_ixT = (int16_t*)b.p[FB_DT_IXT]; h->d_dt_iy = (int16_t*)b.p[FB_DT_IY];
+  h->d_dt_tmpT = b.p[FB_DT_TMPT]; h->d_dt_sdt = b.p[FB_DT_SDT]; h->d_dt_ixT = b.p[FB_DT_IXT]; h->d_dt_iy = b.p[FB_DT_IY]; h->dt_ptr_bytes = lay.ptr_bytes;
   h->d_acc = b.p[FB_ACC]; h->d_feat_split = (uint16_t*)b.p[FB_FEAT_SPLIT];
   h->pyr_launches = std::move(t.pyr_launches);
   if (h->pad == 0) { h->d_hog_levels = h->d_levels; h->d_padjobs = nullptr; h->d_padblocks = nullptr; }
@@ -521,7 +521,7 @@
   }
   launch_backtrack(h->d_cand_count, h->d_cand_rec, h->opt.max_candidates, h->d_back, h->md.ncomponents, h->d_parent,
                    h->d_plane0, h->d_nparts, h->max_parts, h->d_mix_rows, out, h->cand_stride, h->ts, h->d_flat,
-                   h->d_depth, h->max_depth, (int)h->parts.size(), h->d_scr_base, h->d_dt_ixT, h->d_dt_iy,
+                   h->d_depth, h->max_depth, (int)h->parts.size(), h->d_scr_base, h->d_dt_ixT, h->d_dt_iy, h->dt_ptr_bytes,
                    h->opt.dt_correct_ptr, h->ext_ptr ? h->d_extx : nullptr, h->d_exty, h->d_ext_base, count_out, h->pad,
                    h->d_foldjobs, h->ik_lazy && !h->ext_ptr ? h->d_pick : nullptr, h->stream);
   if (post) return pbd_i_post_enqueue(h, cm, zf, out);
@@ -937,21 +937,23 @@
   const size_t po = L.cell_off * h->nplanes + (size_t)(P.plane0 + parent_mix) * HW;
   if (!L.active) return fail(h, PBD_ERR_STATE, "level is not processed by this handle");
   std::vector<uint8_t> c(HW);
-  std::vector<int16_t> X((size_t)P.K * HW), Y((size_t)P.K * HW);
+  const size_t pb = (size_t)h->dt_ptr_bytes;
+  std::vector<uint8_t> X((size_t)P.K * HW * pb), Y((size_t)P.K * HW * pb);
+  auto at = [pb](const std::vector<uint8_t>& v, size_t i) { return pb == 1 ? (int)v[i] : (int)((const int16_t*)v.data())[i]; };
   const size_t so = (size_t)h->scr_base[(size_t)level * h->parts.size() + (p0 + part)];
   ON_DEVICE(h);
   { int rc = ensure_ik(h); if (rc) return rc; }
   HIPCHK(h, hipStreamSynchronize(h->stream));
   HIPCHK(h, hipMemcpy(c.data(), h->d_pk + po, HW, hipMemcpyDeviceToHost));
-  HIPCHK(h, hipMemcpy(X.data(), h->d_dt_ixT + so, X.size() * 2, hipMemcpyDeviceToHost));
-  HIPCHK(h, hipMemcpy(Y.data(), h->d_dt_iy + so, Y.size() * 2, hipMemcpyDeviceToHost));
+  HIPCHK(h, hipMemcpy(X.data(), (const char*)h->d_dt_ixT + so * pb, X.size(), hipMemcpyDeviceToHost));
+  HIPCHK(h, hipMemcpy(Y.data(), (const char*)h->d_dt_iy + so * pb, Y.size(), hipMemcpyDeviceToHost));
   const int W = L.cw, H = L.ch;
   for (size_t i = 0; i < HW; ++i) {
     const size_t mo = (size_t)c[i] * HW;
     const int m_ = (int)(i / W), n_ = (int)(i - (size_t)m_ * W);
     int x, y;
-    if (!h->opt.dt_correct_ptr) { x = X[mo + (size_t)n_ * H + m_]; y = Y[mo + (size_t)m_ * W + x]; }
-    else { y = Y[mo + i]; x = X[mo + (size_t)n_ * H + y]; }
+    if (!h->opt.dt_correct_ptr) { x = at(X, mo + (size_t)n_ * H + m_); y = at(Y, mo + (size_t)m_ * W + x); }
+    else { y = at(Y, mo + i); x = at(X, mo + (size_t)n_ * H + y); }
     if (ix) ix[i] = x;
     if (iy) iy[i] = y;
     if (ik) ik[i] = c[i];
@@ -1171,9 +1173,10 @@
   ON_DEVICE(h);
   const size_t ts = (size_t)tsz;
   char *d_in, *d_tmp, *d_sdt;
-  int16_t *d_ixT, *d_iy;
+  char *d_ixT, *d_iy;
+  const size_t pb = (size_t)dt_ptr_bytes_for(std::max(rows, cols));
   HIPCHK(h, hipMalloc(&d_in, HW * ts)); HIPCHK(h, hipMalloc(&d_tmp, HW * ts)); HIPCHK(h, hipMalloc(&d_sdt, HW * ts));
-  HIPCHK(h, hipMalloc(&d_ixT, HW * 2)); HIPCHK(h, hipMalloc(&d_iy, HW * 2));
+  HIPCHK(h, hipMalloc(&d_ixT, HW * pb)); HIPCHK(h, hipMalloc(&d_iy, HW * pb));
   HIPCHK(h, hipMemcpyAsync(d_in, in, HW * ts, hipMemcpyHostToDevice, h->stream));
   DtMap maps[2] = {dt_map(d_in, d_tmp, d_ixT, 0.f, 0.f, osx, 1), dt_map(d_tmp, d_sdt, d_iy, 0.f, 0.f, osy, 0)};
   maps[0].a = ax; maps[0].b = bx; maps[0].r2a = 1.0 / (2.0 * ax);
@@ -1188,6 +1191,7 @@
   const int nx = (int)tasks.size();
   dt_add_tasks(groups[1], tasks);
   dt_mark_fused(tasks, maps, tsz);
+  if (pb == 1) dt_mark_ptr8(tasks);
   DtMap* d_maps; DtTask* d_tasks;
   HIPCHK(h, hipMalloc(&d_maps, sizeof(maps)));
   HIPCHK(h, hipMalloc(&d_tasks, sizeof(DtTask) * tasks.size()));
@@ -1195,12 +1199,13 @@
   HIPCHK(h, hipMemcpyAsync(d_tasks, tasks.data(), sizeof(DtTask) * tasks.size(), hipMemcpyHostToDevice, h->stream));
   HIPCHK(h, hipStreamSynchronize(h->stream));
   launch_dt_pass(d_tasks, nx, d_maps, nullptr, nullptr, h->d_biasw, budget, tsz, nt, 0, h->stream);
-  if (PBD_PROBE_ENV("PBD_DEBUG_SKIP_Y")) { hipMemsetAsync(d_sdt, 0, HW * ts, h->stream); hipMemsetAsync(d_iy, 0, HW * 2, h->stream); }
+  if (PBD_PROBE_ENV("PBD_DEBUG_SKIP_Y")) { hipMemsetAsync(d_sdt, 0, HW * ts, h->stream); hipMemsetAsync(d_iy, 0, HW * pb, h->stream); }
   else launch_dt_pass(d_tasks + nx, (int)tasks.size() - nx, d_maps, nullptr, nullptr, h->d_biasw, budget, tsz, nt, 0, h->stream);
-  std::vector<int16_t> hx(HW), hy(HW);
+  std::vector<uint8_t> hx(HW * pb), hy(HW * pb);
+  auto at = [pb](const std::vector<uint8_t>& v, size_t i) { return pb == 1 ? (int)v[i] : (int)((const int16_t*)v.data())[i]; };
   HIPCHK(h, hipMemcpyAsync(out, d_sdt, HW * ts, hipMemcpyDeviceToHost, h->stream));
-  HIPCHK(h, hipMemcpyAsync(hx.data(), d_ixT, HW * 2, hipMemcpyDeviceToHost, h->stream));
-  HIPCHK(h, hipMemcpyAsync(hy.data(), d_iy, HW * 2, hipMemcpyDeviceToHost, h->stream));
+  HIPCHK(h, hipMemcpyAsync(hx.data(), d_ixT, HW * pb, hipMemcpyDeviceToHost, h->stream));
+  HIPCHK(h, hipMemcpyAsync(hy.data(), d_iy, HW * pb, hipMemcpyDeviceToHost, h->stream));
   std::vector<char> htmp(HW * ts);
   HIPCHK(h, hipMemcpyAsync(htmp.data(), d_tmp, HW * ts, hipMemcpyDeviceToHost, h->stream));
   HIPCHK(h, hipStreamSynchronize(h->stream));
@@ -1209,8 +1214,8 @@
   for (size_t i = 0; i < HW; ++i) {
     const int m_ = (int)(i / cols), n_ = (int)(i - (size_t)m_ * cols);
     int x, y;
-    if (!h->opt.dt_correct_ptr) { x = hx[(size_t)n_ * rows + m_]; y = hy[(size_t)m_ * cols + x]; }
-    else { y = hy[i]; x = hx[(size_t)n_ * rows + y]; }
+    if (!h->opt.dt_correct_ptr) { x = at(hx, (size_t)n_ * rows + m_); y = at(hy, (size_t)m_ * cols + x); }
+    else { y = at(hy, i); x = at(hx, (size_t)n_ * rows + y); }
     if (ix) ix[i] = x;
     if (iy) iy[i] = y;
   }
diff --git a/partsbaseddetector_amd/csrc/pbd_internal.hpp b/partsbaseddetector_amd/csrc/pbd_internal.hpp
--- a/partsbaseddetector_amd/csrc/pbd_internal.hpp
+++ b/partsbaseddetector_amd/csrc/pbd_internal.hpp
@@ -127,7 +127,7 @@
   int* d_depth = nullptr;
   int max_depth = 0;
   char* d_rootv = nullptr; int* d_rooti = nullptr;
-  char* d_dt_tmpT = nullptr; char* d_dt_sdt = nullptr; int16_t* d_dt_ixT = nullptr; int16_t* d_dt_iy = nullptr;
+  char* d_dt_tmpT = nullptr; char* d_dt_sdt = nullptr; void* d_dt_ixT = nullptr; void* d_dt_iy = nullptr; int dt_ptr_bytes = 2;
   size_t dt_cap_elems = 0;
   LevelDev* d_levels = nullptr;
   LevelDev* d_hog_levels = nullptr;
@@ -430,7 +430,7 @@
 void launch_backtrack(const int* count, const CandRec* rec, int capacity, const BackLevel* back, int ncomp,
                       const int* parent, const int* plane0, const int* nparts, int max_parts, const int* mix_rows,
                       char* out, size_t out_stride, int ts, const int* flat, const int* depth, int max_depth, int nflat,
-                      const unsigned long long* scr_base, const int16_t* ix, const int16_t* iy, int correct_ptr,
+                      const unsigned long long* scr_base, const void* ix, const void* iy, int ptr_bytes, int correct_ptr,
                       const int16_t* extx, const int16_t* exty, const unsigned long long* ext_base, int* count_out, int pad,
                       const FoldJob* folds, const unsigned long long* pick, hipStream_t s);
 void launch_ik_fill(const FoldJob* folds, const unsigned long long* pick, const ReduceBlock* blocks, int nblocks, const unsigned* cells, int ts, hipStream_t s);
diff --git a/partsbaseddetector_amd/csrc/pbd_plan.cpp b/partsbaseddetector_amd/csrc/pbd_plan.cpp
--- a/partsbaseddetector_amd/csrc/pbd_plan.cpp
+++ b/partsbaseddetector_amd/csrc/pbd_plan.cpp
@@ -349,6 +349,11 @@
 }
 
 static bool has_cells(const Level& L) { return L.active && L.cw > 0 && L.ch > 0; }
+static int plan_maxlen(const std::vector<Level>& lv) {
+  int maxlen = 1;
+  for (const Level& L : lv) if (L.active) maxlen = std::max(maxlen, std::max(L.cw, L.ch));
+  return maxlen;
+}
 
 int plan_layout(const HostModel& hm, const FrameSpec& f, FrameLayout& out, std::string* err) {
   const pbd_model_desc& m = hm.md;
@@ -429,6 +434,7 @@
   own(FB_ROOTV, cells * m.ncomponents * ts);
   own(FB_ROOTI, std::max<size_t>(cells * m.ncomponents, 1) * sizeof(int));
   if (hm.nms_sz > 0) own(FB_NMS_MASK, cells * m.ncomponents);
+  out.ptr_bytes = dt_ptr_bytes_for(plan_maxlen(out.lv));
   own(FB_DT_IXT, out.dt_cap_elems * sizeof(int16_t));
   own(FB_DT_IY, out.dt_cap_elems * sizeof(int16_t));
   if (!hm.fold) own(FB_ACC, cells * hm.nslots * ts);
@@ -507,7 +513,11 @@
     if (ok) g.fused |= DT_G_FUSED;
   }
 }
-DtMap dt_map(const void* src, void* dst, int16_t* ptr, float wq, float wl, int os, int natural) {
+int dt_ptr_bytes_for(int maxlen) { return dt_stride_for(maxlen) <= 256 ? 1 : 2; }
+void dt_mark_ptr8(std::vector<DtTask>& tasks) {
+  for (DtTask& t : tasks) t.g.fused |= DT_G_PTR8;
+}
+DtMap dt_map(const void* src, void* dst, void* ptr, float wq, float wl, int os, int natural) {
   DtMap m{};
   m.src = src; m.dst = dst; m.ptr = ptr;
   m.a = -(double)wq; m.b = -(double)wl;
@@ -603,9 +613,8 @@
 }
 
 static int dt_geometry(const HostModel& hm, const FrameLayout& lay, int dt_geom, const PlanKnobs& kn, FrameTables& out, std::string* err) {
-  int maxlen = 1;
-  for (const Level& L : lay.lv) if (L.active) maxlen = std::max(maxlen, std::max(L.cw, L.ch));
-  const bool byte_links = dt_stride_for(maxlen) <= 256;
+  const int maxlen = plan_maxlen(lay.lv);
+  const bool byte_links = lay.ptr_bytes == 1;
   const bool big_blocks = hm.ts == 4 && dt_geom ? dt_geom == 1 : byte_links;
   out.dt_nt = hm.ts == 8 ? 128 : (big_blocks ? 256 : PBD_DT_NT_DEFAULT);
   if (kn.dt_nt) out.dt_nt = kn.dt_nt;
@@ -732,8 +741,8 @@
         const char* src = (!fold && slot_init[P.slot[mm]]) ? pa.acc(l, P.slot[mm]) : pa.resp(l, fid);
         const float* wv = &hm.defw[(size_t)did * 4];
         char* tmp = pa.b.p[FB_DT_TMPT] + to * ts;
-        maps.push_back(dt_map(src, tmp, (int16_t*)pa.b.p[FB_DT_IXT] + so, wv[0], wv[1], hm.anchors[did * 2], 1));
-        ymaps.push_back(dt_map(tmp, pa.sdt(fp, l, mm), (int16_t*)pa.b.p[FB_DT_IY] + so, wv[2], wv[3], hm.anchors[did * 2 + 1], 0));
+        maps.push_back(dt_map(src, tmp, pa.b.p[FB_DT_IXT] + so * (size_t)lay.ptr_bytes, wv[0], wv[1], hm.anchors[did * 2], 1));
+        ymaps.push_back(dt_map(tmp, pa.sdt(fp, l, mm), pa.b.p[FB_DT_IY] + so * (size_t)lay.ptr_bytes, wv[2], wv[3], hm.anchors[did * 2 + 1], 0));
         gx_nmaps++;
       }
       tmp_round += (size_t)P.K;
@@ -746,6 +755,7 @@
   }
   dt_mark_fused(xt, maps.data(), ts);
   dt_mark_fused(yt, maps.data(), ts);
+  if (lay.ptr_bytes == 1) { dt_mark_ptr8(xt); dt_mark_ptr8(yt); }
   xcd_order(xt, kn.xcd_chunk);
   xcd_order(yt, kn.xcd_chunk);
   R.lds_x = launch_lds(xt, ts, nt); R.lds_y = launch_lds(yt, ts, nt); R.fold_x = fold_x ? 1 : 0;
diff --git a/partsbaseddetector_amd/csrc/pbd_plan.hpp b/partsbaseddetector_amd/csrc/pbd_plan.hpp
--- a/partsbaseddetector_amd/csrc/pbd_plan.hpp
+++ b/partsbaseddetector_amd/csrc/pbd_plan.hpp
@@ -37,7 +37,7 @@
 struct DtMap {
   const void* src;
   void* dst;
-  int16_t* ptr;
+  void* ptr;
   double a, b;
   double r2a;
   int os, ptr_natural;
@@ -54,6 +54,7 @@
 };
 #define DT_G_FUSED 1
 #define DT_G_NATURAL 2
+#define DT_G_PTR8 4
 struct DtTask { int g0, nl, m0, l0; DtGroup g;
   const void* src0; };
 static inline unsigned dt_magic(unsigned d) { return d > 1 ? 0xFFFFFFFFu / d + 1u : 0u; }
@@ -187,6 +188,7 @@
   size_t act_cells = 0;
   size_t maxK = 1;
   size_t dt_cap_elems = 0;
+  int ptr_bytes = 2;
   bool compact = false;
   BufPlace buf[FB_COUNT];
   std::vector<size_t> regions;
@@ -237,7 +239,9 @@
                  bool round_lanes = true);
 void dt_add_tasks(const DtGroup& g, std::vector<DtTask>& out, const std::vector<DtMap>* maps = nullptr, int ts = 4);
 void dt_mark_fused(std::vector<DtTask>& tasks, const DtMap* maps, int ts);
-DtMap dt_map(const void* src, void* dst, int16_t* ptr, float wq, float wl, int os, int natural);
+DtMap dt_map(const void* src, void* dst, void* ptr, float wq, float wl, int os, int natural);
+int dt_ptr_bytes_for(int maxlen);
+void dt_mark_ptr8(std::vector<DtTask>& tasks);
 
 int compute_geometry(int w, int h, int sbin, int interval, int* nlevels, Level* lv);
 int compute_geometry_matlab(int w, int h, int sbin, int interval, int* nlevels, Level* lv);
```

After: 2467, median of 6. 2.3% higher.
